# bpatchasaheb/mayaMatchMoveSolver

Hardware: AMD Instinct MI355X
Metric: LM iterations/sec + residuals/sec (markers x frames) at 1/2/4/8 MI355X; final RMS reproj error (higher is better)
Workload: dtype f64; 1 GPU; c4_500pose_50kbnd_200kobs; frames=500, cameras=1, bundles=50000, markers=50000, observations=200000, parameters=152991, residuals=400000, parallelism=single, solver=lmder fwd-FD delta=1e-4 tau=1 tol=1e-6

## Files before the change

include/mmba.h:

```cpp
#ifndef MMBA_H
#define MMBA_H

#include <stddef.h>
#include <stdint.h>

#ifdef __cplusplus
extern "C" {
#endif

#define MMBA_ABI_VERSION 12

#define MMBA_OK 0
#define MMBA_ERR_INVALID (-1)
#define MMBA_ERR_DEVICE (-2)
#define MMBA_ERR_UNSUPPORTED (-3)
#define MMBA_ERR_INTERRUPTED (-4)
#define MMBA_ERR_NO_DEVICE (-5)
#define MMBA_ERR_COMM (-6)

#define MMBA_SOLVER_CMINPACK_LMDIF 1
#define MMBA_SOLVER_CMINPACK_LMDER 2

#define MMBA_SCENE_GRAPH_MAYA_DAG 1
#define MMBA_SCENE_GRAPH_MM_SCENE_GRAPH 2
// ... 226 lines not shown

typedef struct mmba_error_metrics {
    int32_t *frame_count;
    double *frame_avg;
    double *frame_max;
    int32_t *frame_max_marker;
    int32_t *marker_count;
    double *marker_avg;
    double *marker_max;
    int32_t *marker_max_frame;
} mmba_error_metrics;
int mmba_plan_error_metrics(mmba_plan *plan, mmba_error_metrics *out);

int mmba_plan_param_layout(const mmba_plan *plan, int32_t *class_out, int32_t *block_out);

int mmba_solve_per_frame(mmba_context *ctx, const mmba_problem *prob,
                         const mmba_options *opt, double *x_inout,
                         mmba_result *results , int32_t max_concurrency,
                         const mmba_callbacks *cb);

int mmba_plan_solve_per_frame(mmba_plan *plan, double *x_inout, mmba_result *results,
                              const mmba_callbacks *cb);

int mmba_solve(mmba_context *ctx, const mmba_problem *prob,
               const mmba_options *opt, double *x_inout, double *fvec_out,
               double *err_user_out, double *err_dist_out, mmba_result *res,
               const mmba_callbacks *cb, mmba_trace *trace);

typedef struct mmba_kernel_stats {
    double jac_ms_avg;
    double jac_bytes;
    int32_t jac_launches;
    double resid_ms_avg;
    double resid_bytes;
    int32_t resid_launches;
    double chol_ms_avg;
    double chol_flops;
    int32_t chol_launches;
    int32_t reduced_dim;
    int32_t reduced_kind;
    int32_t dataflow_fallback;
    int32_t shards_replicated;
    int32_t spec_replays;
    int32_t band_solver;
    int32_t band_levels;
    int32_t band_block;
    double chol_flops_alg;
    int32_t pre_handbacks;
    int32_t ne_split_launches;
    int32_t trial_red_folds;
} mmba_kernel_stats;
int mmba_plan_kernel_stats(mmba_plan *plan, int enable_timing,
                           mmba_kernel_stats *out);

#define MMBA_PATH_PCR 1
#define MMBA_PATH_SHARD_BCR 2
#define MMBA_PATH_BCR_DATAFLOW 3
#define MMBA_PATH_BCR_GRID 4
#define MMBA_PATH_DENSE 5
#define MMBA_PATH_PERFRAME_BATCH 6
#define MMBA_PATH_LOCAL_RING 7
#define MMBA_PATH_PROBE 8
#define MMBA_PATH_SHARD_SEP 9
#define MMBA_PATH_TRIAL_RECORDS 10
#define MMBA_PATH_LENS_CF 11
#define MMBA_PATH_DEST_LANE 12
#define MMBA_PATH_FAULT_SHARD 13
#define MMBA_PATH_COMM_TIMEOUT_MS 14
#define MMBA_PATH_STALL_SHARD 15
#define MMBA_PATH_PCR_CHAIN 16
#define MMBA_PATH_BACKSUB_ONEPASS 17
#define MMBA_PATH_JB_RECOMPUTE 18
#define MMBA_PATH_NE_CF_SPLIT 19
#define MMBA_PATH_RED_BD 20
#define MMBA_PATH_HANDBACK_DMA 21
#define MMBA_PATH_PRE_HANDBACK 22
#define MMBA_PATH_PRE_SCHUR 23
#define MMBA_PATH_BACKSUB_GROUP 24
#define MMBA_PATH_TRIAL_RED_FOLD 25
#define MMBA_PATH_LENS_SHARED 26
#define MMBA_PATH_OBJ_CF 27
#define MMBA_PATH_OBJ_REC 28
#define MMBA_PATH_PCR_WIDE 29
#define MMBA_PATH_NUM 30
int mmba_debug_set_path(int key, int value);

int mmba_debug_band_solve(mmba_context *ctx, int nb, int w, int nG, int P, const double *S,
                          const double *r, double *x, double *ynorm2, int *parts_used);
int mmba_debug_comm_allreduce(mmba_context *ctx, mmba_comm *comm, double *buf, int count,
                              int op);
int mmba_debug_dgemm(mmba_context *ctx, int tri, int in_place, int M, int N, int K,
                     const double *A, int lda, const double *B, int ldb, double *C, int ldc,
                     double alpha, double beta);

int mmba_debug_reduced_residual(mmba_plan *plan, const double *x, double lam, double *relres);

int mmba_debug_damped_step(mmba_plan *plan, const double *x, double lam, double *step_out,
                           double *g_out, double *diag_out, double *fjac_out);

int mmba_debug_error_metrics(mmba_context *ctx, int32_t num_frames, int32_t num_markers,
                             int32_t num_obs, const int32_t *obs_marker,
                             const int32_t *obs_frame, const double *err_dist,
                             mmba_error_metrics *out);

#ifdef __cplusplus
}
#endif

#endif
```

mayamatchmovesolver_amd/abi.py:

```python
import ctypes as C

MMBA_OK = 0
MMBA_ERR_INVALID = -1
MMBA_ERR_DEVICE = -2
MMBA_ERR_UNSUPPORTED = -3
MMBA_ERR_INTERRUPTED = -4
MMBA_ERR_NO_DEVICE = -5
MMBA_ERR_COMM = -6

SOLVER_TYPE_CMINPACK_LMDIF = 1
SOLVER_TYPE_CMINPACK_LMDER = 2
SCENE_GRAPH_MODE_MAYA_DAG = 1
SCENE_GRAPH_MODE_MM_SCENE_GRAPH = 2
AUTO_DIFF_TYPE_FORWARD = 0
AUTO_DIFF_TYPE_CENTRAL = 1
ROBUST_LOSS_TYPE_TRIVIAL = 0
ROBUST_LOSS_TYPE_SOFT_L_ONE = 1
ROBUST_LOSS_TYPE_CAUCHY = 2
ABI_VERSION = 12

PATH_PCR = 1
PATH_SHARD_BCR = 2
PATH_BCR_DATAFLOW = 3
PATH_BCR_GRID = 4
PATH_DENSE = 5
PATH_PERFRAME_BATCH = 6
PATH_LOCAL_RING = 7
PATH_PROBE = 8
PATH_SHARD_SEP = 9
PATH_TRIAL_RECORDS = 10
PATH_LENS_CF = 11
PATH_DEST_LANE = 12
PATH_FAULT_SHARD = 13
PATH_COMM_TIMEOUT_MS = 14
PATH_STALL_SHARD = 15
PATH_PCR_CHAIN = 16
PATH_BACKSUB_ONEPASS = 17
PATH_JB_RECOMPUTE = 18
PATH_NE_CF_SPLIT = 19
PATH_RED_BD = 20
PATH_HANDBACK_DMA = 21
PATH_PRE_HANDBACK = 22
PATH_PRE_SCHUR = 23
PATH_BACKSUB_GROUP = 24
PATH_TRIAL_RED_FOLD = 25
PATH_LENS_SHARED = 26
PATH_OBJ_CF = 27
PATH_OBJ_REC = 28
PATH_PCR_WIDE = 29
PATH_NUM = 30

FILM_FIT_FILL = 0
FILM_FIT_HORIZONTAL = 1
FILM_FIT_VERTICAL = 2
FILM_FIT_OVERSCAN = 3

ROO_XYZ, ROO_YZX, ROO_ZXY, ROO_XZY, ROO_YXZ, ROO_ZYX = range(6)

LENS_NONE = 0
LENS_3DE_CLASSIC = 1
LENS_3DE_RADIAL_STD_DEG4 = 2
LENS_3DE_ANAMORPHIC_STD_DEG4 = 3
LENS_3DE_ANAMORPHIC_STD_DEG4_RESCALED = 4

CAM_FILM_BACK_W_INCH = 0
CAM_FILM_BACK_H_INCH = 1
CAM_FOCAL_MM = 2
CAM_FILM_OFFSET_X_INCH = 3
CAM_FILM_OFFSET_Y_INCH = 4
CAM_NEAR_CLIP = 5
CAM_FAR_CLIP = 6
CAM_SCALE = 7
CAM_NUM_ATTRS = 8
LENS_NUM_ATTRS = 14

_i32p = C.POINTER(C.c_int32)
_i64p = C.POINTER(C.c_int64)
_f64p = C.POINTER(C.c_double)


class MmbaProblem(C.Structure):
    _fields_ = [
        ("num_frames", C.c_int32),
        ("num_attrs", C.c_int32),
        ("attr_animated", _i32p),
        ("attr_offset", _i64p),
        ("attr_values", _f64p),
        ("num_transforms", C.c_int32),
        ("tfm_parent", _i32p),
        ("tfm_rotate_order", _i32p),
        ("tfm_attrs", _i32p),
        ("num_cameras", C.c_int32),
        ("cam_tfm", _i32p),
        ("cam_attrs", _i32p),
        ("cam_film_fit", _i32p),
        ("cam_render_size", _i32p),
        ("cam_lens", _i32p),
        ("num_lenses", C.c_int32),
        ("lens_type", _i32p),
        ("lens_attrs", _i32p),
        ("num_bundles", C.c_int32),
        ("bnd_tfm", _i32p),
        ("num_markers", C.c_int32),
        ("mkr_cam", _i32p),
        ("mkr_bnd", _i32p),
        ("num_obs", C.c_int32),
        ("obs_marker", _i32p),
        ("obs_frame", _i32p),
        ("obs_xy", _f64p),
        ("obs_weight", _f64p),
        ("num_params", C.c_int32),
        ("param_attr", _i32p),
        ("param_frame", _i32p),
        ("param_min", _f64p),
        ("param_max", _f64p),
        ("param_offset", _f64p),
        ("param_scale", _f64p),
        ("param_weight", _f64p),
        ("num_stiff", C.c_int32),
        ("stiff_attr", _i32p),
        ("stiff_frame", _i32p),
        ("stiff_weight", _f64p),
        ("stiff_variance", _f64p),
        ("stiff_value", _f64p),
        ("num_smooth", C.c_int32),
        ("smooth_attr", _i32p),
        ("smooth_frame", _i32p),
        ("smooth_weight", _f64p),
        ("smooth_variance", _f64p),
        ("smooth_value", _f64p),
        ("cam_rs_value", _f64p),
        ("lens_input", _i32p),
        ("lens_input_values", _f64p),
# ... 166 lines not shown
```

mayamatchmovesolver_amd/csrc/mmba_api.cpp:

```cpp
#include <atomic>
#include <cfloat>
#include <cmath>
#include <cstring>
#include <string>

#include "mmba_geom.h"
#include "mmba_kernels.h"
#include "mmba_plan.h"

namespace mmba {
static thread_local std::string g_last_error;
void set_error(const std::string &msg) { g_last_error = msg; }

static_assert(MMBA_PATH_NUM == 30, "one initialiser per path key");
static std::atomic<int> g_path[MMBA_PATH_NUM] = {-1, -1, -1, -1, -1, -1, -1, -1, -1, -1, -1, -1, -1,
                                                 -1, -1, -1, -1, -1, -1, -1, -1, -1, -1, -1, -1,
                                                 -1, -1, -1, -1, -1};
int path_choice(int key) {
    return (key > 0 && key < MMBA_PATH_NUM) ? g_path[key].load() : -1;
}
}

using namespace mmba;

#define MMBA_GUARD(...)                               \
    try {                                             \
        __VA_ARGS__                                   \
    } catch (const DeviceError &) {                   \
        return MMBA_ERR_DEVICE;                       \
    } catch (const CommError &) {                     \
        return MMBA_ERR_COMM;                         \
    } catch (const Unsupported &u) {                  \
        set_error("unsupported: " + u.what);          \
        return MMBA_ERR_UNSUPPORTED;                  \
    } catch (const Invalid &v) {                      \
        set_error("invalid: " + v.what);              \
        return MMBA_ERR_INVALID;                      \
    } catch (const std::exception &e) {               \
        set_error(std::string("exception: ") + e.what()); \
        return MMBA_ERR_INVALID;                      \
    }

extern "C" {

int mmba_abi_version(void) { return MMBA_ABI_VERSION; }

int mmba_debug_set_path(int key, int value) {
    if (key <= 0 || key >= MMBA_PATH_NUM) return MMBA_ERR_INVALID;
    g_path[key].store(value < 0 ? -1 : value);
    return MMBA_OK;
}

int mmba_shard_layout(int32_t num_frames, int32_t num_obs, const int32_t *obs_frame,
                      const int32_t *obs_bundle, int32_t num_bundles, int32_t nranks,
                      int32_t *bounds_out, int32_t *bundle_owner_out) {
    if (num_frames <= 0 || num_obs < 0 || nranks <= 0 || !bounds_out ||
        (num_obs > 0 && !obs_frame) || (bundle_owner_out && (!obs_bundle || num_bundles < 0)))
        return MMBA_ERR_INVALID;
    for (int i = 0; i < num_obs; ++i) {
        if (obs_frame[i] < 0 || obs_frame[i] >= num_frames) return MMBA_ERR_INVALID;
        if (bundle_owner_out && (obs_bundle[i] < 0 || obs_bundle[i] >= num_bundles))
            return MMBA_ERR_INVALID;
    }
    mmba::shard_layout(num_frames, num_obs, obs_frame, obs_bundle, num_bundles, nranks,
                       bounds_out, bundle_owner_out);
    return MMBA_OK;
}

const char *mmba_last_error(void) { return g_last_error.c_str(); }

int mmba_device_count(void) {
    int count = 0;
    if (hipGetDeviceCount(&count) != hipSuccess) return 0;
    int ok = 0;
    for (int d = 0; d < count; ++d) {
        hipDeviceProp_t prop;
        if (hipGetDeviceProperties(&prop, d) != hipSuccess) continue;
        if (std::strncmp(prop.gcnArchName, "gfx950", 6) == 0) ++ok;
    }
    return ok;
}

void mmba_options_default(mmba_options *o, int32_t solver_type) {
    if (!o) return;
    std::memset(o, 0, sizeof(*o));
    o->solver_type = solver_type ? solver_type : MMBA_SOLVER_CMINPACK_LMDER;
    o->iter_max = 100;
    o->tau = 1.0;
    o->eps1 = 1e-6;
    o->eps2 = 1e-6;
    o->eps3 = 1e-6;
    o->delta = 1e-4;
    o->auto_diff_type = MMBA_AUTO_DIFF_FORWARD;
    o->auto_param_scale = 1;
    o->scene_graph_mode = MMBA_SCENE_GRAPH_MAYA_DAG;
    o->image_width = 2048.0;
    o->accept_only_better = 1;
    o->log_level = 0;
}

// ... 576 lines not shown
```

mayamatchmovesolver_amd/csrc/mmba_internal.h:

```cpp
#pragma once

#include <hip/hip_runtime.h>
#include <stdint.h>

#include <string>
#include <vector>

#include "../../include/mmba.h"

namespace mmba {

constexpr int PCMAX = 12;
constexpr int PBMAX = 3;
constexpr int NGMAX = 48;
constexpr int NGLANE = 16;
constexpr int NGPART = 32;
constexpr int LMAX = 32;
constexpr int CF_AIDX = 16;
constexpr int TILE = 64;
constexpr int CAMREC = 20;
constexpr int LENS_LAYER = 1 + MMBA_LENS_NUM_ATTRS;
constexpr int LENS_CHAIN_MAX = 4;
constexpr int BREC = 16;
constexpr int ORECSZ = 12;
// ... 100 lines not shown
    int s_xn2 = 0, s_gnorm = 0, s_f0 = 0, s_out = 0;
    int *gate = nullptr;
};
struct BandSolver {
    bool use_bd = false;
    BdDev bd;
    bool use_bcr = false;
    BcrDev bcr;
    bool use_pcr = false;
    PcrDev pcr;
    mutable unsigned tick_f = 0, tick_b = 0;
    mutable bool df_off = false;
    int df_grid = 256;
    double *red = nullptr, *red_rhs = nullptr;
    size_t red_count = 0;
    int P = 1, w = 0, nb = 0, nG = 0;
    int p_lo = 0, p_hi = 1;
    Comm *comm = nullptr;
    long long max_arrow = 0;
    double *Bd = nullptr, *Ga = nullptr, *Gd = nullptr, *Gdinv = nullptr, *Dinv = nullptr;
    BandPart *d_parts = nullptr;
    double *apool = nullptr, *zpool = nullptr, *cpool = nullptr;
    double *TBd = nullptr, *TGa = nullptr, *TGd = nullptr, *TGdinv = nullptr, *TDinv = nullptr;
    size_t tcount = 0;
    BandPart *d_tpart = nullptr;
    double *rT = nullptr, *yT = nullptr, *xT = nullptr;
    bool pcr_int = false;
    PcrDev ipcr;
    BandPart hpart{};
    double *XA = nullptr, *izero = nullptr, *ix = nullptr;
    int *fail = nullptr;
};

struct SView {
    int band;
    int dense, ld;
    double *S;
    const int *slot;
    int NT;
    double *Bd;
    int w, nb;
    double *Ga;
    double *Gd;
};

enum ParamClass : int { PC_CF = 0, PC_B = 1, PC_G = 2 };

enum VarFlags : int { VF_BUNDLE_SIDE = 1, VF_LENS = 2, VF_OBJ = 4 };

struct DevProblem {
    int F, nA, nT, nC, nL, nB, nK, M, n, ncf, nR, nG, mode;
    int nbs;
    double image_width;
    const int64_t *attr_off;
    const int *attr_anim;
    double *attr_val;
    const int *tfm_parent, *tfm_roo, *tfm_attrs;
    const int *cam_tfm, *cam_attrs, *cam_fit, *cam_size, *cam_lens;
    const int *lens_attrs, *lens_type;
    const double *lens_chain;
    int lens_chain_n;
    int lens_uniform;
    const int *bnd_tfm;
    const int *obs_cf, *obs_bnd, *obs_frame, *obs_cam;
    const double *obs_xy, *obs_sqrtw;
    const int *cf_cam, *cf_frame, *cf_obs_off, *cf_var_off, *cf_var_param, *cf_var_flags;
    const int *cf_pc, *cf_roff;
    int pc_uniform;
    int wst;
    int dest_diag_ii;
    const int *bnd_par_off, *bnd_par;
    const int *bnd_pb;
    const int *bnd_xoff;
    const int *bobs_off, *bobs;
    const int4 *bnd_p4;
    const double *brec;
    int all_bnd_fast;
    int lmax;
    int jcol_implicit;
    const int *cf_aidx;
    int no_lens;
    const int *obs_bpos;
    double *JB;
    const int *cam_lpar_off, *cam_lpar;
    const int *obs_inst, *inst_lens, *inst_attr, *inst_frame, *inst_lpar_off, *inst_lpar;
    const double *inst_val;
    const int *p_attr, *p_frame, *p_class, *p_pos, *p_both, *p_blk;
    const double *p_min, *p_max, *p_off, *p_scale;
    const int *g_param;
    const int *obs_own, *cf_own, *bnd_own;
    int root, Ra, Rb;
    int nrows, rows_live;
    const int *row_attr, *row_frame, *row_param;
    const double *row_w, *row_var, *row_val;
    int loss_on, loss_type;
    double loss_scale;
    const long long *p_vidx;
    const int4 *bnd_vx;
    const int *bnd_pcomp;
    int rs;
    const double *obs_tau;
    const int *cf_rs_nb, *cf_rs_vidx;
    const int *cf_rs_gcnt, *cf_rs_gcol, *cf_rs_gidx;
    double *rs_Aoff;
    int ls_ng, ls_nl;
    const int *ls_tab;
    double *ls_Aoff;
};

struct ObjRecDev {
    int n = 0;
    const int *obs_set = nullptr, *off = nullptr, *par = nullptr, *set = nullptr, *tf = nullptr;
    double *rec = nullptr;
};
struct NoObjRec {};

__device__ __forceinline__ size_t widx(const DevProblem &P, int k, int i) {
    return (size_t)i * P.wst + k;
}

__device__ __forceinline__ double *s_at(const SView &V, int R, int C) {
    if (V.dense) return &V.S[(size_t)C * V.ld + R];
    if (!V.band) {
        const int s = V.slot[(R / TILE) * V.NT + (C / TILE)];
        return &V.S[(size_t)s * TILE * TILE + (R % TILE) * TILE + (C % TILE)];
    }
    if (R < V.nb) return &V.Bd[(size_t)R * (V.w + 1) + (C - R + V.w)];
    if (C < V.nb) return &V.Ga[(size_t)(R - V.nb) * V.nb + C];
    return &V.Gd[(R - V.nb) * NGMAX + (C - V.nb)];
}

}
```

mayamatchmovesolver_amd/csrc/mmba_kernels.h:

```cpp
#pragma once

#include <vector>

#include "mmba_internal.h"

namespace mmba {

constexpr int NE_BND_TPB = 64;

inline int nblk(long n, int bs) { return (int)((n + bs - 1) / bs); }

void launch_param_set(hipStream_t s, const DevProblem &P, const double *x, double *ext,
                      double *ext_pert, double *step, int solver_type, double delta,
                      double eps_dif);
struct RedRow {
    int off, n, is_max, slot;
};
struct RedSpec {
    int nrows;
    int flag_slot;
    RedRow row[8];
};
void launch_reduce_multi(hipStream_t s, const double *partial, const RedSpec &spec,
                         double *scalar, int *flag = nullptr, double *host = nullptr,
// ... 21 lines not shown
                          const double *recs, double *f, double *eu, double *ed, double *partial,
                          double *out, unsigned int *ticket, double *dist);
void launch_residual_jp_orec(hipStream_t s, const DevProblem &P, const ObjRecDev &O,
                             const double *recs, double *f, double *eu, double *ed,
                             double *partial, const double *J, const int *jcol, const int *nloc,
                             const double *pstep, double *partial_jp, double *dist);
void launch_jacobian_orec(hipStream_t s, const DevProblem &P, const ObjRecDev &O,
                          const double *recs, const double *ext_pert, const double *step,
                          int solver_type, double *J, int *jcol, int *nloc,
                          const int *stale_param, double *eu, double *ed);
int residual_blocks(const DevProblem &P);
bool &trial_cf_off();
int trial_blocks(const DevProblem &P);
void launch_reproject(hipStream_t s, const DevProblem &P, const double *recs, double *pts,
                      double *mkr);
void launch_residual(hipStream_t s, const DevProblem &P, const double *recs, double *f, double *eu,
                     double *ed, double *partial, double *out = nullptr,
                     unsigned int *ticket = nullptr, double *dist = nullptr,
                     const ObjRecDev *O = nullptr);
void launch_dist_stats(hipStream_t s, const DevProblem &P, const double *ed, double *partial,
                       int nparts, int rstride, double *out);
void launch_residual_jp(hipStream_t s, const DevProblem &P, const double *recs, double *f,
                        double *eu, double *ed, double *partial, const double *J,
                        const int *jcol, const int *nloc, const double *pstep,
                        double *partial_jp, double *dist = nullptr,
                        const ObjRecDev *O = nullptr);
struct CentralB {
    const double *recs = nullptr, *brec = nullptr, *ext_pert = nullptr, *step = nullptr;
    const double *q15 = nullptr, *kap15 = nullptr;
};
void launch_param_central(hipStream_t s, const DevProblem &P, const double *x, double *ext_pertB,
                          double *stepB, double delta, double *count, double *c15 = nullptr);
void launch_b15_s(hipStream_t s, const double *fsq, double fn, double *out);
void launch_b15_combine(hipStream_t s, int n, const double *u, const double *c, const double *zu,
                        const double *zc, const double *sp, double *xs, double *kinv,
                        double *scalar, int fail_slot, const double *fail_prev);
void launch_b15_q(hipStream_t s, const DevProblem &P, const double *c, double *q15, double *kap15,
                  double *cr);
void launch_b15_rot(hipStream_t s, const DevProblem &P, const double *q15, const double *x,
                    double *out);
void launch_b15_accl(hipStream_t s, const DevProblem &P, const double *Acc, const double *q15,
                     const double *diag, double lam, double *AccL, double *diagL);
void launch_b15_unrot(hipStream_t s, const DevProblem &P, const double *Acc, const double *g,
                      const double *q15, double *adiag, double *u);
void launch_b15_unrot_J(hipStream_t s, const DevProblem &P, double *J, const double *q15);
void launch_b15_dnorm(hipStream_t s, int n, const double *x, const double *diag, double *out);
void launch_b15_newton(hipStream_t s, int n, const double *v, const double *zu, const double *zc,
                       const double *kinv, double *out);
void launch_b15_jp(hipStream_t s, int n, const double *xs, const double *u, const double *c,
                   const double *sp, double *out);
void launch_jacobian(hipStream_t s, const DevProblem &P, const double *recs,
                     const double *ext_pert, const double *step, int solver_type, double *J,
                     int *jcol, int *nloc, const int *stale_param, double *eu, double *ed,
                     int ncv = 0,
                     const double *f = nullptr,
                     const CentralB &CB = CentralB(),
                     const ObjRecDev *O = nullptr);
void launch_rows_eval(hipStream_t s, const DevProblem &P, double *fr, double *eur,
                      double *partial, int slot, const double *Jrow = nullptr,
                      const double *pstep = nullptr, double *partial_jp = nullptr);
void launch_rows_jac(hipStream_t s, const DevProblem &P, const double *ext,
                     const double *ext_pert, const double *step, const double *ext_pertB,
                     const double *stepB, int lmder, double *Jrow, double *eur, int last_param);
void launch_rows_ne(hipStream_t s, const DevProblem &P, const double *Jrow, const double *fr,
                    const int *p_own, double *Acc, double *Abb, double *aggbuf, double *g);
constexpr int NE_CF_SPLIT = 4;
constexpr int NE_CF_NT = 36;
struct NeEpi {
    int on = 0;
    int first = 0, mode = 1, do_xn = 0, do_gn = 0;
    double fnorm = 0.;
    const double *fnorm_sq = nullptr;
    const double *x = nullptr;
    double *diag = nullptr, *acnorm = nullptr, *partial = nullptr;
    int rstride = 0, cf_base = 0, bnd_base = 0;
    const double *jb_recs = nullptr;
    int jb_lmder = 1;
    double *cf_part = nullptr;
    unsigned *cf_ticket = nullptr;
    double *Lb = nullptr, *tb = nullptr;
    int *fail = nullptr;
    const int *gate = nullptr;
    long long *probe = nullptr;
};
struct TrialRed {
    int on = 0;
    RedSpec spec{};
    LmDec dec{};
    const double *partial = nullptr;
    double *scalar = nullptr;
    double *host = nullptr;
    int host_n = 0;
    unsigned *host_seq = nullptr;
    unsigned seq = 0;
};
bool jac_ne_fusable(const DevProblem &P, int ncv);
void launch_jac_ne(hipStream_t s, const DevProblem &P, const double *recs, const double *step,
                   int solver_type, double *J, int *jcol, int *nloc, const int *stale_param,
                   double *eu, double *ed, double *Acc, double *g, const NeEpi &E,
                   const TrialRed &R = TrialRed());
bool ne_epilogue_fusable(const DevProblem &P);
bool launch_ne(hipStream_t s, const DevProblem &P, const double *J, const int *jcol,
               const int *nloc, const double *f, double *Acc, double *Acg, double *Abb,
               double *Abg, double *aggbuf, double *g, double *glob_partial, int glob_chunk,
               const NeEpi &epi = NeEpi(), bool cf_done = false);
void launch_colnorms(hipStream_t s, const DevProblem &P, const double *Acc, const double *Abb,
                     const double *aggbuf, double *acnorm, double *g);
void launch_bundle_factor(hipStream_t s, const DevProblem &P, const double *Abb,
                          const double *Abg, const double *g, const double *diag, double lam,
                          double *Lb, double *tb, double *Wg, int *fail);
void launch_schur_obs(hipStream_t s, const DevProblem &P, const double *J, const double *Lb,
                      double *W, const RedSpec *red = nullptr, const double *partial = nullptr,
                      double *scalar = nullptr, const int *gate = nullptr);
void launch_schur_obs_rs(hipStream_t s, const DevProblem &PV, int Mr, const int *nloc,
                         const int *vobs, const int *vcoff, const double *J, const double *Lb,
                         double *W);
void launch_schur_init(hipStream_t s, const DevProblem &P, const double *Acc, const double *Acg,
                       const double *Agg, const double *g, const double *diag, double lam,
                       const SView &V, int npad, double *rhs, const RedSpec *red = nullptr,
                       const double *partial = nullptr, double *scalar = nullptr);
void launch_schur_pairs(hipStream_t s, const DevProblem &P, const double *W, const double *Wg,
                        const double *tb, const SView &V, double *rhs);
void launch_chol_panel(hipStream_t s, double *S, const int *slot, int NT, int k, const int *rows,
                       int nrows, double *Linv, int *fail);
void launch_chol_update(hipStream_t s, double *S, const int *slot, int NT, int k,
                        const int2 *pairs, int npairs);
void launch_trsv_fwd(hipStream_t s, const double *S, const int *slot, int NT, int k,
                     const int *rows, int nrows, const double *Linv, double *r, double *y);
void launch_trsv_bwd(hipStream_t s, const double *S, const int *slot, int NT, int k,
                     const int *cols, int ncols, const double *Linv, double *y, double *x);
void launch_trsv_fwd_all(hipStream_t s, const double *S, const int *slot, int NT,
                         const int *rows_off, const int *rows, const double *Linv, double *r,
                         double *y);
void launch_trsv_bwd_all(hipStream_t s, const double *S, const int *slot, int NT,
                         const int *cols_off, const int *cols, const double *Linv, double *y,
                         double *x);
struct SchurInitFold {
    int on;
    const double *Acc, *g, *diag;
    double lam;
};
bool launch_schur_dest(hipStream_t s, const DevProblem &P, const double *W, const int2 *dest,
                       const int *dest_off, int ndest, const int2 *pairs, const SView &V,
                       int pc_uniform, int assign_off, const double *tb = nullptr,
                       double *rhs = nullptr, SchurInitFold fold = SchurInitFold{},
                       const int *wave_list = nullptr, int n_wave = 0,
                       const int *lane_list = nullptr, int n_lane = 0);
void launch_schur_rhs(hipStream_t s, const DevProblem &P, const double *W, const double *tb,
                      double *rhs);
void launch_schur_glob(hipStream_t s, const DevProblem &P, const double *W, const double *Wg,
                       const double *tb, const SView &V, double *rhs);
void launch_backsub_bundle(hipStream_t s, const DevProblem &P, const double *W, const double *Wg,
                           const double *tb, const double *Lb, const double *xR, double *U,
                           double *x);
struct TrialFold {
    const double *x = nullptr, *diag = nullptr;
    double *wa1 = nullptr, *wa2 = nullptr, *wa3 = nullptr;
    double *ext = nullptr, *ext_pert = nullptr, *step = nullptr;
    int solver_type = 0;
    double delta = 0., eps_dif = 0.;
    const int *other = nullptr;
    int nother = 0;
    double *partial = nullptr;
    int rstride = 0;
    const int *own = nullptr;
    int rec = 0;
    double *recs = nullptr, *brec = nullptr;
    int group = 0;
    const int2 *bobs_rp = nullptr;
    int brec_fwd = 0;
    int *flag = nullptr;
    double *flag_out = nullptr;
};
bool trial_records_ok(const DevProblem &P);
int trial_fold_parts(const DevProblem &P, int nother, bool rec = false);
int trial_prep_rec_parts(const DevProblem &P, int nother);
void launch_trial_prep_rec(hipStream_t s, const DevProblem &P, const double *xs, const TrialFold &T);
void launch_obs_wtx(hipStream_t s, const DevProblem &P, const double *W, const double *xR,
                    double *U);
void launch_backsub_trial(hipStream_t s, const DevProblem &P, const double *W, const double *Wg,
                          const double *tb, const double *Lb, const double *xR, const double *U,
                          double *x, const TrialFold &T);
void launch_scatter_xR(hipStream_t s, const DevProblem &P, const double *xR, double *x);
void launch_newton_bundle(hipStream_t s, const DevProblem &P, const double *W, const double *Wg,
                          const double *Lb, const double *v, double *wR, double *usq,
                          double *un, double *gp);
void launch_gather_R(hipStream_t s, const DevProblem &P, const double *v, double *vR, int nRpad);
void band_factor(hipStream_t s, const BandSolver &B, int *fail, long long *probe);
void band_factor_forward(hipStream_t s, const BandSolver &B, int *fail, long long *probe,
                         const double *r, double *y);
void band_forward(hipStream_t s, const BandSolver &B, const double *r, double *y);
void band_backward(hipStream_t s, const BandSolver &B, const double *y, double *x);
void bcr_factor(hipStream_t s, const BandSolver &B, int *fail, long long *probe,
                const double *r = nullptr, double *y = nullptr);
void bcr_forward(hipStream_t s, const BandSolver &B, const double *r, double *y);
void bcr_backward(hipStream_t s, const BandSolver &B, const double *y, double *x);
// ... 69 lines not shown
```

mayamatchmovesolver_amd/csrc/mmba_kernels.hip:

```cpp
#include <cfloat>
#include <cstdlib>
#include <type_traits>

#include "mmba_geom.h"
#include "mmba_kernels.h"
#include "mmba_obs_dev.h"
#include "mmba_red_dev.h"

namespace mmba {

__device__ __forceinline__ void bundle_chol3(double (&A)[3][3], double (&rhs)[3],
                                             const double (&dd)[3], int pb, double lam, int b,
                                             double *Lb, double *tb, int *fail,
                                             double (*Lo)[3] = nullptr, double *ilo = nullptr) {
#pragma unroll
    for (int a = 0; a < 3; ++a) {
        if (a < pb) {
            const double d = dd[a];
            A[a][a] += lam * (d * d);
            if (A[a][a] == 0.) {
                A[a][a] = 1.;
                rhs[a] = 0.;
            }
        }
// ... 599 lines not shown
            for (int t = threadIdx.x; t < lm * NE_CHUNK; t += blockDim.x) {
                const int l = t / NE_CHUNK, o = t % NE_CHUNK;
                if (o >= cnt || l < pc || l >= nloc[c0 + o]) continue;
                const int p = jcol[(size_t)l * M + c0 + o];
                if (P.p_class[p] == PC_G) sG[P.p_pos[p] - nCF][o] = l;
            }
        }
        for (int t = threadIdx.x; t < NE_CHUNK; t += blockDim.x) {
            sF[0][t] = (t < cnt) ? f[2 * (c0 + t)] : 0.;
            sF[1][t] = (t < cnt) ? f[2 * (c0 + t) + 1] : 0.;
        }
        __syncthreads();
        if (kind == 0) {
            for (int o = 0; o < cnt; ++o)
                acc += sJ[2 * ea][o] * sJ[2 * eb][o] + sJ[2 * ea + 1][o] * sJ[2 * eb + 1][o];
        } else if (kind == 1) {
            for (int o = 0; o < cnt; ++o)
                acc += sJ[2 * ea][o] * sF[0][o] + sJ[2 * ea + 1][o] * sF[1][o];
        } else if (kind == 2) {
            for (int o = 0; o < cnt; ++o) {
                const int l = sG[eb][o];
                if (l >= 0)
                    acc += sJ[2 * ea][o] * sJ[2 * l][o] + sJ[2 * ea + 1][o] * sJ[2 * l + 1][o];
            }
        }
    }
    double *A = &Acc[(size_t)cf * PCMAX * PCMAX];
    if (kind == 0) {
        A[ea * PCMAX + eb] = acc;
        A[eb * PCMAX + ea] = acc;
    } else if (kind == 1) {
        g[P.cf_var_param[P.cf_var_off[cf] + 1 + ea]] = acc;
    } else if (kind == 2) {
        Acg[((size_t)cf * PCMAX + ea) * NGMAX + eb] = acc;
    }
}

__device__ __forceinline__ double epi_param(const NeEpi &E, int p, double d, double gp, double &zf,
                                          double &xn, double &gm) {
    const double an = sqrt(d);
    E.acnorm[p] = an;
    double dg = E.diag[p];
    if (E.mode != 2) {
        if (E.first) dg = an == 0. ? 1. : an;
        dg = fmax(dg, an);
        E.diag[p] = dg;
    }
    if (an == 0.) zf = 1.;
    if (E.do_xn) {
        const double v = dg * E.x[p];
        xn += v * v;
    }
    if (E.do_gn && an != 0.) {
        const double fn = E.fnorm_sq ? sqrt(*E.fnorm_sq) : E.fnorm;
        if (fn != 0.) gm = fmax(gm, fabs((gp / fn) / an));
    }
    return dg;
}

__device__ __forceinline__ void epi_store(const NeEpi &E, int col, double zf, double xn,
                                          double gm) {
    E.partial[col] = zf;
    E.partial[E.rstride + col] = xn;
    E.partial[2 * E.rstride + col] = gm;
}

struct EpiPre {
    int p;
    double dg;
    double xv;
    double fn;
};
template <int PC>
__device__ __forceinline__ EpiPre epi_preload(const DevProblem &P, const NeEpi &E, int cf,
                                              int lane, bool own = false, double fsq_own = 0.) {
    EpiPre q{-1, 0., 0., 0.};
    if (!E.on || lane >= PC) return q;
    q.p = P.cf_var_param[P.cf_var_off[cf] + 1 + lane];
    q.dg = E.diag[q.p];
    if (E.do_xn) q.xv = E.x[q.p];
    if (E.do_gn) q.fn = own ? sqrt(fsq_own) : E.fnorm_sq ? sqrt(*E.fnorm_sq) : E.fnorm;
    return q;
}
__device__ __forceinline__ void epi_param_pre(const NeEpi &E, const EpiPre &q, double d, double gp,
                                              double &zf, double &xn, double &gm) {
    const double an = sqrt(d);
    E.acnorm[q.p] = an;
    double dg = q.dg;
    if (E.mode != 2) {
        if (E.first) dg = an == 0. ? 1. : an;
        dg = fmax(dg, an);
        E.diag[q.p] = dg;
    }
    if (an == 0.) zf = 1.;
    if (E.do_xn) {
        const double v = dg * q.xv;
        xn += v * v;
    }
    if (E.do_gn && an != 0.) {
        if (q.fn != 0.) gm = fmax(gm, fabs((gp / q.fn) / an));
    }
}
template <int PC>
__device__ __forceinline__ void epi_params_wave(const DevProblem &P, const NeEpi &E, int cf,
                                                int lane, double d, double gp, const EpiPre &q) {
    double zf = 0., xn = 0., gm = 0.;
    if (lane < PC) epi_param_pre(E, q, d, gp, zf, xn, gm);
    double Z = 0., X = 0., G = 0.;
#pragma unroll
    for (int a = 0; a < PC; ++a) {
        const double za = __shfl(zf, a), xa = __shfl(xn, a), ga = __shfl(gm, a);
        if (za != 0.) Z = 1.;
        X += xa;
        G = fmax(G, ga);
    }
    if (lane == 0) epi_store(E, E.cf_base + cf, Z, X, G);
}


template <int PC, int NW, int NG>
__device__ __forceinline__ void ne_cf_u_body(const DevProblem &P, const double *__restrict__ J,
                                             const int *__restrict__ jcol,
                                             const int *__restrict__ nloc,
                                             const double *__restrict__ f, double *Acc,
                                             double *Acg, double *g, const NeEpi &E, int blk,
                                             int nblk_cf) {
    constexpr int NCC = PC * (PC + 1) / 2, NE = NCC + PC, NT = NE + PC * NG;
    __shared__ double wsum[NW][NT];
    const int cf = xcd_remap(blk, nblk_cf);
    if (!own_cf(P, cf) || P.cf_pc[cf] != PC) {
        if (E.on && threadIdx.x == 0) epi_store(E, E.cf_base + cf, 0., 0., 0.);
        return;
    }
    const int o0 = P.cf_obs_off[cf], o1 = P.cf_obs_off[cf + 1];
    const size_t M = P.M;
    const int nCF = P.nR - P.nG;
    const int tid = threadIdx.x, lane = tid & 63, wv = tid >> 6;
    const EpiPre epq = epi_preload<PC>(P, E, cf, lane);
    double acc[NT];
#pragma unroll
    for (int e = 0; e < NT; ++e) acc[e] = 0.;
    for (int i = o0 + tid; i < o1; i += 64 * NW) {
        double jx[PC], jy[PC];
#pragma unroll
        for (int a = 0; a < PC; ++a) {
            jx[a] = J[(2 * a) * M + i];
            jy[a] = J[(2 * a + 1) * M + i];
        }
        const double fx = f[2 * i], fy = f[2 * i + 1];
        int e = 0;
#pragma unroll
        for (int a = 0; a < PC; ++a)
#pragma unroll
            for (int c = a; c < PC; ++c) acc[e++] += jx[a] * jx[c] + jy[a] * jy[c];
#pragma unroll
        for (int a = 0; a < PC; ++a) acc[NCC + a] += jx[a] * fx + jy[a] * fy;
        if constexpr (NG > 0) {
            double gx[NG], gy[NG];
#pragma unroll
            for (int q = 0; q < NG; ++q) gx[q] = gy[q] = 0.;
            const int nl = nloc[i];
            for (int l = PC; l < nl; ++l) {
                const int p = jcol[(size_t)l * M + i];
                if (P.p_class[p] != PC_G) continue;
                const int gi = P.p_pos[p] - nCF;
                const double ux = J[(size_t)(2 * l) * M + i], uy = J[(size_t)(2 * l + 1) * M + i];
#pragma unroll
                for (int q = 0; q < NG; ++q) {
                    gx[q] = (gi == q) ? ux : gx[q];
                    gy[q] = (gi == q) ? uy : gy[q];
                }
            }
#pragma unroll
            for (int a = 0; a < PC; ++a)
#pragma unroll
                for (int q = 0; q < NG; ++q)
                    acc[NE + a * NG + q] += jx[a] * gx[q] + jy[a] * gy[q];
        }
    }
#pragma unroll
    for (int e = 0; e < NT; ++e) {
        double v = acc[e];
#pragma unroll
        for (int off = 32; off > 0; off >>= 1) v += __shfl_xor(v, off);
// ... 137 lines not shown
template <int PC, int NW, int NG>
__global__ void __launch_bounds__(64 * NW) k_ne_cf_u(DevProblem P, const double *__restrict__ J,
                                                     const int *__restrict__ jcol,
                                                     const int *__restrict__ nloc,
                                                     const double *__restrict__ f, double *Acc,
                                                     double *Acg, double *g, NeEpi E) {
    ne_cf_u_body<PC, NW, NG>(P, J, jcol, nloc, f, Acc, Acg, g, E, blockIdx.x, gridDim.x);
}



__device__ __forceinline__ void jac_ne_publish(const TrialRed &R, const LmIn &v, const LmOut &o) {
    if (threadIdx.x == 0) {
        const double val[5] = {v.pnorm, v.xn2t, v.fnorm, v.jp, v.dnorm};
#pragma unroll
        for (int r = 0; r < 5; ++r)
            if (r < R.spec.nrows) R.scalar[R.spec.row[r].slot] = val[r];
        lm_publish(R.dec, o, R.scalar);
    }
    if (!R.host) return;
    if (threadIdx.x < 64) {
        __builtin_amdgcn_fence(__ATOMIC_SEQ_CST, "workgroup");
        for (int i = threadIdx.x; i < R.host_n; i += 64)
            R.host[i] = __hip_atomic_load(&R.scalar[i], __ATOMIC_RELAXED, __HIP_MEMORY_SCOPE_AGENT);
        if (R.host_seq) {
            __threadfence_system();
            if (threadIdx.x == 0)
                __hip_atomic_store(R.host_seq, R.seq, __ATOMIC_RELEASE, __HIP_MEMORY_SCOPE_SYSTEM);
        }
    }
}

struct TrialRows {
    RowQ Q0, Q1;
    int r0, nred;
    bool dn_dup;
};
template <int NW>
__device__ __forceinline__ void trial_rows_issue(const TrialRed &R, LmIn &tin, TrialRows &T) {
    const LmDec &d = R.dec;
    const int nr = R.spec.nrows;
    T.dn_dup = nr == 5 && R.spec.row[4].off == R.spec.row[0].off &&
               R.spec.row[4].n == R.spec.row[0].n &&
               R.spec.row[4].is_max == R.spec.row[0].is_max;
    T.nred = T.dn_dup ? 4 : nr;
    T.r0 = __builtin_amdgcn_readfirstlane((int)threadIdx.x >> 6);
    if (T.r0 < T.nred) row_issue(R.partial, R.spec.row[T.r0], T.Q0);
    if constexpr (NW == 2)
        if (T.r0 + NW < T.nred) row_issue(R.partial, R.spec.row[T.r0 + NW], T.Q1);
    tin.f0 = R.scalar[d.s_f0];
    tin.xn2 = R.scalar[d.s_xn2];
    tin.gnorm = R.scalar[d.s_gnorm];
    tin.fail = R.scalar[d.s_fail];
    if (nr < 5) tin.dnorm = R.scalar[d.s_dnorm];
}
template <int NW>
__device__ __forceinline__ void trial_rows_finish(const TrialRed &R, double *sTr,
                                                  const TrialRows &T) {
    const bool l0 = (threadIdx.x & 63) == 0;
    if (T.r0 < T.nred) {
        const double v = row_finish(R.partial, R.spec.row[T.r0], T.Q0);
        if (l0) sTr[T.r0] = v;
    }
    if constexpr (NW == 2)
        if (T.r0 + NW < T.nred) {
            const double v = row_finish(R.partial, R.spec.row[T.r0 + NW], T.Q1);
            if (l0) sTr[T.r0 + NW] = v;
        }
    for (int r = T.r0 + (NW == 2 ? 2 : 1) * NW; r < T.nred; r += NW) {
        const double v = reduce_row_w64(R.partial, R.spec.row[r]);
        if (l0) sTr[r] = v;
    }
}
__device__ __forceinline__ LmOut trial_decide(const TrialRed &R, const double *sTr, LmIn &tin,
                                              bool dn_dup) {
    tin.pnorm = sTr[0];
    tin.xn2t = sTr[1];
    tin.fnorm = sTr[2];
    tin.jp = sTr[3];
    if (R.spec.nrows == 5) tin.dnorm = dn_dup ? sTr[0] : sTr[4];
    return lm_decide_vals(R.dec, tin);
}

template <int PC, int NW, bool GEN>
__global__ void __launch_bounds__(64 * NW) k_jac_ne_u(
    DevProblem P, const double *__restrict__ recs, const double *__restrict__ step,
    int solver_type, double *__restrict__ J, int *__restrict__ jcol, int *__restrict__ nloc,
    const int *__restrict__ stale_param, double *__restrict__ eu, double *__restrict__ ed,
    double *Acc, double *g, NeEpi E, TrialRed R) {
    constexpr int NCC = PC * (PC + 1) / 2, NE = NCC + PC;
    __shared__ double wsum[NW][NE];
    __shared__ double sRec[(PC + 1) * CAMREC];
    __shared__ int sPv[PC];
    __shared__ double sSt[PC];
    __shared__ int sHdr[3];
    __shared__ double sTr[5];
    if (!R.on && E.gate &&
        __hip_atomic_load(E.gate, __ATOMIC_RELAXED, __HIP_MEMORY_SCOPE_AGENT) == 0)
        return;
    const int tid = threadIdx.x, lane = tid & 63, wv = tid >> 6;
    LmIn tin{};
    TrialRows TR;
    TR.dn_dup = false;
    const int pad = R.on ? 8 : 0;
    const int ncf = (int)gridDim.x - pad;
    if ((int)blockIdx.x < pad) {
        if (blockIdx.x != 0) return;
        trial_rows_issue<NW>(R, tin, TR);
        trial_rows_finish<NW>(R, sTr, TR);
        __syncthreads();
        const LmOut out = trial_decide(R, sTr, tin, TR.dn_dup);
        jac_ne_publish(R, tin, out);
        return;
    }
    const int cf = xcd_remap((int)blockIdx.x - pad, ncf);
    long long *pr = (E.probe && threadIdx.x == 0) ? E.probe + 5 * (size_t)cf : nullptr;
    const long long t_in = pr ? (long long)wall_clock64() : 0;
    const int o0 = P.cf_obs_off[cf], o1 = P.cf_obs_off[cf + 1];
    const bool lmder = solver_type == MMBA_SOLVER_CMINPACK_LMDER;
    const bool solved = P.cf_pc[cf] == PC && own_cf(P, cf);
    {
        constexpr int KT = ((PC + 1) * CAMREC + 64 * NW - 1) / (64 * NW);
        const int voff = P.cf_var_off[cf];
        const int nv = min(P.cf_var_off[cf + 1] - voff - 1, PC);
        double rv[KT];
#pragma unroll
        for (int k = 0; k < KT; ++k) {
            const int t = tid + 64 * NW * k;
            rv[k] = t < (nv + 1) * CAMREC ? recs[(size_t)voff * CAMREC + t] : 0.;
        }
        const int p = (tid < PC && tid < nv) ? P.cf_var_param[voff + 1 + tid] : -1;
        const int fr = P.cf_frame[cf];
        if (R.on) trial_rows_issue<NW>(R, tin, TR);
        const double stv = p >= 0 ? step[p] : 1.;
#pragma unroll
        for (int k = 0; k < KT; ++k) {
            const int t = tid + 64 * NW * k;
            if (t < (nv + 1) * CAMREC) sRec[t] = rv[k];
        }
        if (tid < PC) {
            sPv[tid] = p;
            sSt[tid] = stv;
        }
        if (tid == 0) {
            sHdr[0] = nv;
            sHdr[1] = fr;
            sHdr[2] = stale_param[fr];
        }
    }
    if (R.on) trial_rows_finish<NW>(R, sTr, TR);
    __syncthreads();
    if (R.on && trial_decide(R, sTr, tin, TR.dn_dup).go == 0) return;
    if (pr) {
        pr[0] = t_in;
        pr[1] = (long long)wall_clock64();
    }
    JacCf<PC> C;
    C.rcf = sRec;
#pragma unroll
    for (int v = 0; v < PC; ++v) {
        C.pv[v] = sPv[v];
        C.st[v] = sSt[v];
    }
    C.nv = sHdr[0];
    C.fr = sHdr[1];
    C.pstale = sHdr[2];
    double acc[NE];
#pragma unroll
    for (int e = 0; e < NE; ++e) acc[e] = 0.;
    for (int i = o0 + tid; i < o1; i += 64 * NW) {
        double jx[PC], jy[PC], fx, fy;
        int z = 0;
        asm volatile("" : "+s"(z));
        C.rcf = sRec + z;
        jac_obs_u<PC, GEN>(P, i, C, lmder, J, jcol, nloc, eu, ed, jx, jy, fx, fy);
        int e = 0;
#pragma unroll
        for (int a = 0; a < PC; ++a)
#pragma unroll
            for (int c = a; c < PC; ++c) acc[e++] += jx[a] * jx[c] + jy[a] * jy[c];
#pragma unroll
        for (int a = 0; a < PC; ++a) acc[NCC + a] += jx[a] * fx + jy[a] * fy;
    }
    if (pr) pr[2] = (long long)wall_clock64();
    if (!solved) {
        if (E.on && tid == 0) epi_store(E, E.cf_base + cf, 0., 0., 0.);
        if (pr) pr[3] = pr[2];
        return;
    }
#pragma unroll
    for (int e = 0; e < NE; ++e) {
        double v = acc[e];
#pragma unroll
        for (int off = 32; off > 0; off >>= 1) v += __shfl_xor(v, off);
        if (lane == 0) wsum[wv][e] = v;
    }
    __syncthreads();
    double *A = &Acc[(size_t)cf * PCMAX * PCMAX];
    for (int e = tid; e < NE; e += 64 * NW) {
        double v = wsum[0][e];
#pragma unroll
        for (int w = 1; w < NW; ++w) v += wsum[w][e];
        if (e < NCC) {
            int a = 0, rem = e;
            while (rem >= PC - a) {
                rem -= PC - a;
                ++a;
            }
            const int c = a + rem;
            A[a * PCMAX + c] = v;
            A[c * PCMAX + a] = v;
        } else {
            g[P.cf_var_param[P.cf_var_off[cf] + 1 + (e - NCC)]] = v;
        }
    }
    if (E.on && (tid >> 6) == 0) {
        const int ln = tid & 63;
        double d = 0., gp = 0.;
        if (ln < PC) {
            const int ed2 = ln * PC - ln * (ln - 1) / 2;
            d = wsum[0][ed2];
            gp = wsum[0][NCC + ln];
#pragma unroll
            for (int w = 1; w < NW; ++w) {
                d += wsum[w][ed2];
                gp += wsum[w][NCC + ln];
            }
        }
        epi_params_wave<PC>(P, E, cf, ln, d, gp, epi_preload<PC>(P, E, cf, ln, R.on != 0, sTr[2]));
    }
    if (pr) {
        pr[3] = (long long)wall_clock64();
        unsigned xcc;
        asm volatile("s_getreg_b32 %0, hwreg(HW_REG_XCC_ID)" : "=s"(xcc));
        pr[4] = (long long)(xcc & 0xf);
    }
}

__global__ void __launch_bounds__(NE_BND_TPB) k_ne_bnd_jb(DevProblem P, double *Abb, double *g,
                                                          NeEpi E) {
    __shared__ double red[3][NE_BND_TPB];
    if (E.gate && __hip_atomic_load(E.gate, __ATOMIC_RELAXED, __HIP_MEMORY_SCOPE_AGENT) == 0)
        return;
    const int b = xcd_remap(blockIdx.x, gridDim.x) * blockDim.x + threadIdx.x;
    const int4 p4 = b < P.nB ? P.bnd_p4[b] : make_int4(-1, -1, -1, 0);
    const int pb = p4.w;
    double zf = 0., xn = 0., gm = 0.;
    if (pb > 0) {
        double A[PBMAX][PBMAX] = {};
        double gb[PBMAX] = {};
        const int q0 = P.bobs_off[b], q1 = P.bobs_off[b + 1];
        const double *__restrict__ br = &P.brec[(size_t)b * BREC];
        for (int qb = q0; qb < q1; qb += 4) {
            double4 u[4], v[4];
            if (E.jb_recs) {
                const double bp0[3] = {br[0], br[1], br[2]};
#pragma unroll
                for (int r = 0; r < 4; ++r) {
                    if (qb + r >= q1) break;
                    const int i = P.bobs[qb + r];
                    const double *__restrict__ rec0 = &E.jb_recs[(size_t)P.cf_var_off[P.obs_cf[i]] * CAMREC];
                    const double mx = P.obs_xy[2 * i], my = P.obs_xy[2 * i + 1], sw = P.obs_sqrtw[i];
                    const double2 f0 = residual_e(rec0, bp0, mx, my, sw, P.mode, P.image_width);
                    double jb[6] = {0., 0., 0., 0., 0., 0.};
#pragma unroll
                    for (int a = 0; a < 3; ++a) {
                        if (a < pb) {
                            const double bq[3] = {br[3 + 3 * a], br[4 + 3 * a], br[5 + 3 * a]};
                            const double2 rr = residual_e(rec0, bq, mx, my, sw, P.mode, P.image_width);
                            const double st = br[12 + a];
                            jb[2 * a] = E.jb_lmder ? (rr.x - f0.x) * st : (rr.x - f0.x) / st;
                            jb[2 * a + 1] = E.jb_lmder ? (rr.y - f0.y) * st : (rr.y - f0.y) / st;
                        }
                    }
                    u[r] = make_double4(jb[0], jb[1], jb[2], jb[3]);
                    v[r] = make_double4(jb[4], jb[5], f0.x, f0.y);
                }
            } else {
#pragma unroll
                for (int r = 0; r < 4; ++r) {
                    if (qb + r < q1) {
                        const double4 *src = reinterpret_cast<const double4 *>(&P.JB[(size_t)(qb + r) * 8]);
                        u[r] = src[0];
                        v[r] = src[1];
                    }
                }
            }
#pragma unroll
            for (int r = 0; r < 4; ++r) {
                if (qb + r >= q1) break;
                const double jx[3] = {u[r].x, u[r].z, v[r].x}, jy[3] = {u[r].y, u[r].w, v[r].y};
                const double fx = v[r].z, fy = v[r].w;
#pragma unroll
                for (int a = 0; a < 3; ++a) {
#pragma unroll
                    for (int c = 0; c < 3; ++c) A[a][c] += jx[a] * jx[c] + jy[a] * jy[c];
                    gb[a] += jx[a] * fx + jy[a] * fy;
                }
            }
        }
        double *Ab = &Abb[(size_t)b * 9];
#pragma unroll
        for (int a = 0; a < PBMAX; ++a)
#pragma unroll
            for (int c = 0; c < PBMAX; ++c) Ab[a * 3 + c] = (a < pb && c < pb) ? A[a][c] : 0.;
        g[p4.x] = gb[0];
        if (pb > 1) g[p4.y] = gb[1];
        if (pb > 2) g[p4.z] = gb[2];
        double dd[3] = {0., 0., 0.};
        if (E.on) {
            double zo = 0., xo = 0., go = 0.;
            dd[0] = epi_param(E, p4.x, A[0][0], gb[0], zo, xo, go);
            if (pb > 1) dd[1] = epi_param(E, p4.y, A[1][1], gb[1], zo, xo, go);
            if (pb > 2) dd[2] = epi_param(E, p4.z, A[2][2], gb[2], zo, xo, go);
            if (own_bnd(P, b)) {
                zf = zo;
                xn = xo;
                gm = go;
            }
        }
        if (E.Lb) {
            double Af[3][3], rhs[3];
#pragma unroll
            for (int a = 0; a < 3; ++a) {
#pragma unroll
                for (int c = 0; c < 3; ++c)
                    Af[a][c] = (a < pb && c < pb) ? A[a][c] : (a == c ? 1. : 0.);
                rhs[a] = a < pb ? gb[a] : 0.;
            }
            bundle_chol3(Af, rhs, dd, pb, 0.0, b, E.Lb, E.tb, E.fail);
        }
    }
    if (!E.on) return;
    red[0][threadIdx.x] = zf;
    red[1][threadIdx.x] = xn;
    red[2][threadIdx.x] = gm;
    __syncthreads();
    for (int w = NE_BND_TPB / 2; w > 0; w >>= 1) {
        if (threadIdx.x < w) {
            red[0][threadIdx.x] = fmax(red[0][threadIdx.x], red[0][threadIdx.x + w]);
            red[1][threadIdx.x] += red[1][threadIdx.x + w];
            red[2][threadIdx.x] = fmax(red[2][threadIdx.x], red[2][threadIdx.x + w]);
        }
        __syncthreads();
    }
    if (threadIdx.x == 0) {
        const int col = E.bnd_base + xcd_remap(blockIdx.x, gridDim.x);
        epi_store(E, col, red[0][0], red[1][0], red[2][0]);
    }
}

__global__ void k_ne_bnd(DevProblem P, const double *__restrict__ J,
                         const int *__restrict__ jcol, const int *__restrict__ nloc,
                         const double *__restrict__ f, double *Abb, double *Abg, double *g) {
    const int b = blockIdx.x * blockDim.x + threadIdx.x;
    if (b >= P.nB) return;
    const int pb = P.bnd_pb[b];
    if (pb == 0) return;
    const int M = P.M, nG = P.nG;
    double A[PBMAX][PBMAX] = {};
    double gb[PBMAX] = {};
    double G[PBMAX][NGMAX];
    for (int a = 0; a < PBMAX; ++a)
        for (int q = 0; q < NGMAX; ++q) G[a][q] = 0.;
    for (int q = P.bobs_off[b]; q < P.bobs_off[b + 1]; ++q) {
        const int i = P.bobs[q];
        const int cf = P.obs_cf[i];
        const int s = P.rs ? nloc[i] - pb : P.cf_var_off[cf + 1] - P.cf_var_off[cf] - 1;
        double jx[PBMAX], jy[PBMAX];
        for (int a = 0; a < pb; ++a) {
            jx[a] = J[(size_t)(2 * (s + a)) * M + i];
            jy[a] = J[(size_t)(2 * (s + a) + 1) * M + i];
        }
        const double fx = f[2 * i], fy = f[2 * i + 1];
        for (int a = 0; a < pb; ++a) {
            for (int c = 0; c < pb; ++c) A[a][c] += jx[a] * jx[c] + jy[a] * jy[c];
            gb[a] += jx[a] * fx + jy[a] * fy;
        }
        if (nG > 0) {
            const int nl = nloc[i];
            for (int l = 0; l < nl; ++l) {
                const int p = jcol[(size_t)l * M + i];
                if (P.p_class[p] != PC_G) continue;
                const int gi = P.p_pos[p] - (P.nR - nG);
                const double gx = J[(size_t)(2 * l) * M + i], gy = J[(size_t)(2 * l + 1) * M + i];
                for (int a = 0; a < pb; ++a) G[a][gi] += jx[a] * gx + jy[a] * gy;
            }
        }
    }
    double *Ab = &Abb[(size_t)b * 9];
    for (int a = 0; a < PBMAX; ++a)
        for (int c = 0; c < PBMAX; ++c) Ab[a * 3 + c] = (a < pb && c < pb) ? A[a][c] : 0.;
    const int po = P.bnd_par_off[b];
    for (int a = 0; a < pb; ++a) g[P.bnd_par[po + a]] = gb[a];
    for (int a = 0; a < PBMAX; ++a)
        for (int q = 0; q < nG; ++q) Abg[((size_t)b * PBMAX + a) * NGMAX + q] = G[a][q];
}
// ... 314 lines not shown
                                                      double *host, int host_n,
                                                      unsigned *ticket, unsigned *host_seq,
                                                      unsigned seq, const LmDec dec) {
    __shared__ double red[256];
    const RedRow rw = spec.row[blockIdx.x];
    const double v = reduce_row_block<false>(partial, rw, red);
    if (threadIdx.x == 0) {
        scalar[rw.slot] = v;
        if (blockIdx.x == 0 && flag && spec.flag_slot >= 0) {
            scalar[spec.flag_slot] = (double)*flag;
            *flag = 0;
        }
    }
    if (!host && !dec.on) return;
    __shared__ unsigned last;
    if (threadIdx.x == 0) {
        const unsigned t = __hip_atomic_fetch_add(ticket, 1u, __ATOMIC_ACQ_REL,
                                                  __HIP_MEMORY_SCOPE_AGENT);
        last = t == gridDim.x - 1;
    }
    __syncthreads();
    if (!last) return;
    __builtin_amdgcn_fence(__ATOMIC_ACQUIRE, "agent");
    if (dec.on) {
        if (threadIdx.x == 0) lm_decide(dec, scalar);
        __syncthreads();
        __builtin_amdgcn_fence(__ATOMIC_SEQ_CST, "workgroup");
    }
    if (!host) {
        if (threadIdx.x == 0)
            __hip_atomic_store(ticket, 0u, __ATOMIC_RELAXED, __HIP_MEMORY_SCOPE_AGENT);
        return;
    }
    if (threadIdx.x < 64) {
        for (int i = threadIdx.x; i < host_n; i += 64)
            host[i] = __hip_atomic_load(&scalar[i], __ATOMIC_RELAXED, __HIP_MEMORY_SCOPE_AGENT);
        if (host_seq) {
            __threadfence_system();
            if (threadIdx.x == 0)
                __hip_atomic_store(host_seq, seq, __ATOMIC_RELEASE, __HIP_MEMORY_SCOPE_SYSTEM);
        }
    }
    if (threadIdx.x == 0) __hip_atomic_store(ticket, 0u, __ATOMIC_RELAXED, __HIP_MEMORY_SCOPE_AGENT);
}

__global__ void k_bundle_factor(DevProblem P, const double *__restrict__ Abb,
                                const double *__restrict__ Abg, const double *__restrict__ g,
                                const double *__restrict__ diag, double lam, double *Lb,
                                double *tb, double *Wg, int *fail) {
    const int b = xcd_remap(blockIdx.x, gridDim.x) * blockDim.x + threadIdx.x;
    if (b >= P.nB) return;
    const int pb = P.bnd_pb[b];
    if (pb == 0) return;
    const int po = P.bnd_par_off[b];
    double A[3][3], rhs[3], dd[3];
#pragma unroll
    for (int a = 0; a < 3; ++a) {
#pragma unroll
        for (int c = 0; c < 3; ++c)
            A[a][c] = (a < pb && c < pb) ? Abb[(size_t)b * 9 + a * 3 + c] : (a == c ? 1. : 0.);
        rhs[a] = 0.;
        dd[a] = 0.;
        if (a < pb) {
            const int p = P.bnd_par[po + a];
            dd[a] = diag[p];
            rhs[a] = g[p];
        }
    }
    double L[3][3], il[3];
    bundle_chol3(A, rhs, dd, pb, lam, b, Lb, tb, fail, L, il);
    for (int q = 0; q < P.nG; ++q) {
        double w[3];
#pragma unroll
        for (int a = 0; a < 3; ++a) {
            double s = a < pb ? Abg[((size_t)b * PBMAX + a) * NGMAX + q] : 0.;
#pragma unroll
            for (int k = 0; k < a; ++k) s -= L[a][k] * w[k];
            w[a] = s * il[a];
        }
        for (int a = 0; a < 3; ++a) Wg[((size_t)b * NGMAX + q) * 3 + a] = w[a];
    }
}

template <int PCT>
__global__ void __launch_bounds__(64) k_schur_obs(DevProblem P, const double *__restrict__ J,
                                                  const double *__restrict__ Lb, double *W,
                                                  int nob, const RedSpec red,
                                                  const double *__restrict__ partial,
                                                  double *scalar, const int *gate) {
    extern __shared__ double sw[];
    if (gate && __hip_atomic_load(gate, __ATOMIC_RELAXED, __HIP_MEMORY_SCOPE_AGENT) == 0) return;
    const int lane = threadIdx.x;
    if ((int)blockIdx.x >= nob) {
        const RedRow rw = red.row[blockIdx.x - nob];
        const double v = reduce_row_w64(partial, rw);
        if (lane == 0) scalar[rw.slot] = v;
        return;
    }
    const int i0 = xcd_remap(blockIdx.x, nob) * 64;
    const int i = i0 + lane;
    const int M = P.M, wst = P.wst;
    double *row = &sw[lane * wst];
    for (int k = 0; k < wst; ++k) row[k] = 0.;
    const int b = i < M ? P.obs_bnd[i] : 0;
    const int pb = i < M ? P.bnd_pb[b] : 0;
    if (pb > 0) {
        const int cf = P.obs_cf[i];
        const int pc = min(min(P.cf_pc[cf], wst / 3), PCT);
        const int s = P.cf_var_off[cf + 1] - P.cf_var_off[cf] - 1;
        double bx[3], by[3], L[3][3], il[3];
#pragma unroll
        for (int a = 0; a < 3; ++a) {
            bx[a] = a < pb ? J[(size_t)(2 * (s + a)) * M + i] : 0.;
            by[a] = a < pb ? J[(size_t)(2 * (s + a) + 1) * M + i] : 0.;
#pragma unroll
            for (int c = 0; c < 3; ++c) L[a][c] = Lb[(size_t)b * 9 + a * 3 + c];
        }
#pragma unroll
        for (int a = 0; a < 3; ++a) il[a] = a < pb ? 1.0 / L[a][a] : 0.;
        double cx[PCT], cy[PCT];
#pragma unroll
        for (int r = 0; r < PCT; ++r) {
            cx[r] = r < pc ? J[(size_t)(2 * r) * M + i] : 0.;
            cy[r] = r < pc ? J[(size_t)(2 * r + 1) * M + i] : 0.;
        }
#pragma unroll
        for (int r = 0; r < PCT; ++r) {
            if (r < pc) {
                double w[3];
#pragma unroll
                for (int a = 0; a < 3; ++a) {
                    double t = cx[r] * bx[a] + cy[r] * by[a];
#pragma unroll
                    for (int k = 0; k < a; ++k) t -= L[a][k] * w[k];
                    w[a] = t * il[a];
                }
#pragma unroll
                for (int a = 0; a < 3; ++a) row[r * 3 + a] = w[a];
            }
        }
    }
    __syncthreads();
    const int nrow = min(64, M - i0);
    const size_t base = (size_t)i0 * wst;
    if (wst % 2 == 0) {
        const int nv = nrow * wst / 2;
        double2 *dst = reinterpret_cast<double2 *>(&W[base]);
        const double2 *src = reinterpret_cast<const double2 *>(sw);
        for (int k = lane; k < nv; k += 64) dst[k] = src[k];
    } else {
        for (int k = lane; k < nrow * wst; k += 64) W[base + k] = sw[k];
    }
}

__global__ void __launch_bounds__(64) k_schur_obs_rs(DevProblem PV, int Mr,
                                                     const int *__restrict__ nloc,
                                                     const int *__restrict__ vobs,
                                                     const int *__restrict__ vcoff,
                                                     const double *__restrict__ J,
                                                     const double *__restrict__ Lb, double *W) {
    const int v = blockIdx.x * blockDim.x + threadIdx.x;
    if (v >= PV.M) return;
    const int wst = PV.wst;
    double *row = &W[(size_t)v * wst];
    for (int k = 0; k < wst; ++k) row[k] = 0.;
    const int b = PV.obs_bnd[v];
    const int pb = PV.bnd_pb[b];
    if (pb <= 0) return;
    const int i = vobs[v], cf = PV.obs_cf[v];
    const int pc = min(PV.cf_pc[cf], wst / 3);
    const int c0 = vcoff[v], s = nloc[i] - pb;
    double bx[3], by[3], L[3][3], il[3];
#pragma unroll
    for (int a = 0; a < 3; ++a) {
        bx[a] = a < pb ? J[(size_t)(2 * (s + a)) * Mr + i] : 0.;
        by[a] = a < pb ? J[(size_t)(2 * (s + a) + 1) * Mr + i] : 0.;
#pragma unroll
        for (int c = 0; c < 3; ++c) L[a][c] = Lb[(size_t)b * 9 + a * 3 + c];
    }
#pragma unroll
    for (int a = 0; a < 3; ++a) il[a] = a < pb ? 1.0 / L[a][a] : 0.;
    for (int r = 0; r < pc; ++r) {
        const double cx = J[(size_t)(2 * (c0 + r)) * Mr + i], cy = J[(size_t)(2 * (c0 + r) + 1) * Mr + i];
        double w[3];
#pragma unroll
        for (int a = 0; a < 3; ++a) {
            double t = cx * bx[a] + cy * by[a];
#pragma unroll
            for (int k = 0; k < a; ++k) t -= L[a][k] * w[k];
            w[a] = t * il[a];
        }
#pragma unroll
        for (int a = 0; a < 3; ++a) row[r * 3 + a] = w[a];
    }
}

__device__ __forceinline__ void schur_init_row(
    const DevProblem &P, const double *__restrict__ Acc, const double *__restrict__ Acg,
    const double *__restrict__ Agg, const double *__restrict__ g,
// ... 1406 lines not shown
        nmn = fmax(nmn, partial[rstride + i]);
        mx = fmax(mx, partial[2 * rstride + i]);
    }
    red[0][threadIdx.x] = sm;
    red[1][threadIdx.x] = nmn;
    red[2][threadIdx.x] = mx;
    __syncthreads();
    for (int w = 128; w > 0; w >>= 1) {
        if ((int)threadIdx.x < w) {
            red[0][threadIdx.x] += red[0][threadIdx.x + w];
            red[1][threadIdx.x] = fmax(red[1][threadIdx.x], red[1][threadIdx.x + w]);
            red[2][threadIdx.x] = fmax(red[2][threadIdx.x], red[2][threadIdx.x + w]);
        }
        __syncthreads();
    }
    if (threadIdx.x == 0) {
        out[0] = red[0][0];
        out[1] = red[1][0];
        out[2] = red[2][0];
    }
}

void launch_dist_stats(hipStream_t s, const DevProblem &P, const double *ed, double *partial,
                       int nparts, int rstride, double *out) {
    k_dist_stats<<<nparts, 256, 0, s>>>(P, ed, partial, rstride);
    k_dist_stats_fin<<<1, 256, 0, s>>>(partial, nparts, rstride, out);
}
void launch_jacobian(hipStream_t s, const DevProblem &P, const double *recs,
                     const double *ext_pert, const double *step, int solver_type, double *J,
                     int *jcol, int *nloc, const int *stale_param, double *eu, double *ed,
                     int ncv, const double *f, const CentralB &CB, const ObjRecDev *O) {
    (void)f;
    if (P.rs) {
        launch_jacobian_rs(s, P, ext_pert, step, solver_type, J, jcol, nloc, stale_param, eu, ed);
        return;
    }
    constexpr bool uni = true;
#define MMBA_JAC_U(NCV, GEN)                                                                \
    do {                                                                                    \
        if (uni)                                                                            \
            k_jacobian_u<NCV, GEN, true><<<nblk(P.M, 128), 128, 0, s>>>(                    \
                P, recs, step, solver_type, J, jcol, nloc, stale_param, eu, ed);            \
        else                                                                                \
            k_jacobian_u<NCV, GEN, false><<<nblk(P.M, 128), 128, 0, s>>>(                   \
                P, recs, step, solver_type, J, jcol, nloc, stale_param, eu, ed);            \
    } while (0)
    if (ncv == 6 || ncv == 7) {
        if (ncv == 6) {
            if (P.all_bnd_fast) MMBA_JAC_U(6, false); else MMBA_JAC_U(6, true);
        } else {
            if (P.all_bnd_fast) MMBA_JAC_U(7, false); else MMBA_JAC_U(7, true);
        }
        return;
    }
#undef MMBA_JAC_U
    if (CB.recs)
        k_jacobian<true><<<nblk(P.M, 128), 128, 0, s>>>(P, recs, ext_pert, step, solver_type, J,
                                                      jcol, nloc, stale_param, eu, ed, CB,
                                                      NoObjRec{});
    else if (O && O->n > 0)
        launch_jacobian_orec(s, P, *O, recs, ext_pert, step, solver_type, J, jcol, nloc,
                             stale_param, eu, ed);
    else if (P.lens_uniform == MMBA_LENS_3DE_CLASSIC)
        k_jacobian<false, MMBA_LENS_3DE_CLASSIC><<<nblk(P.M, 128), 128, 0, s>>>(
            P, recs, ext_pert, step, solver_type, J, jcol, nloc, stale_param, eu, ed, CB,
                                                      NoObjRec{});
    else
        k_jacobian<false><<<nblk(P.M, 128), 128, 0, s>>>(P, recs, ext_pert, step, solver_type, J,
                                                       jcol, nloc, stale_param, eu, ed, CB,
                                                      NoObjRec{});
}
bool jac_ne_fusable(const DevProblem &P, int ncv) {
    return P.nG == 0 && P.pc_uniform == ncv && (ncv == 6 || ncv == 7) &&
           P.nrows == 0 && !P.loss_on && P.ncf >= 256 && !P.rs && !P.ls_ng;
}
void launch_jac_ne(hipStream_t s, const DevProblem &P, const double *recs, const double *step,
                   int solver_type, double *J, int *jcol, int *nloc, const int *stale_param,
                   double *eu, double *ed, double *Acc, double *g, const NeEpi &E,
                   const TrialRed &R) {
    if (P.ncf == 0) return;
    const int grid = P.ncf + (R.on ? 8 : 0);
    const long long per = (P.M + P.ncf - 1) / P.ncf;
    int nw = per > 1024 ? 8 : (per > 256 ? 4 : 2);
#define MMBA_JN(PC, NW, GEN)                                                                  \
    k_jac_ne_u<PC, NW, GEN><<<grid, 64 * NW, 0, s>>>(P, recs, step, solver_type, J, jcol, nloc, \
                                                       stale_param, eu, ed, Acc, g, E, R)
#define MMBA_JN_NW(PC, GEN)                                         \
    do {                                                            \
        if (nw == 8) MMBA_JN(PC, 8, GEN);                           \
        else if (nw == 4) MMBA_JN(PC, 4, GEN);                      \
        else MMBA_JN(PC, 2, GEN);                                   \
    } while (0)
#define MMBA_JN_PC(PC)                                              \
    do {                                                            \
        if (P.all_bnd_fast) MMBA_JN_NW(PC, false);                  \
        else MMBA_JN_NW(PC, true);                                  \
    } while (0)
    if (P.pc_uniform == 6)
        MMBA_JN_PC(6);
    else
        MMBA_JN_PC(7);
#undef MMBA_JN_PC
#undef MMBA_JN_NW
#undef MMBA_JN
}
__global__ void k_fold_ranks(const double *__restrict__ t, int nranks, double *out, int do_xn,
                             int do_gn) {
    if (threadIdx.x != 0) return;
    out[0] = t[0];
    if (do_xn) out[1] = t[1];
    if (do_gn) {
        double g = 0.;
        for (int r = 0; r < nranks; ++r) g = fmax(g, t[2 + r]);
        out[2] = g;
    }
}
void launch_fold_ranks(hipStream_t s, const double *t, int nranks, double *out, int do_xn,
                       int do_gn) {
    k_fold_ranks<<<1, 64, 0, s>>>(t, nranks, out, do_xn, do_gn);
}
void launch_param_central(hipStream_t s, const DevProblem &P, const double *x, double *ext_pertB,
                          double *stepB, double delta, double *count, double *c15) {
    if (P.n > 0)
        k_param_central<<<nblk(P.n, 256), 256, 0, s>>>(P, x, ext_pertB, stepB, delta, count,
                                                        c15);
}

template <int NV>
__device__ __forceinline__ void b15_block_sum(double (&v)[NV], double (*red)[1024]) {
    const int tid = threadIdx.x;
#pragma unroll
    for (int k = 0; k < NV; ++k) red[k][tid] = v[k];
    __syncthreads();
    for (int w = 512; w > 0; w >>= 1) {
        if (tid < w) {
#pragma unroll
            for (int k = 0; k < NV; ++k) red[k][tid] += red[k][tid + w];
        }
        __syncthreads();
    }
#pragma unroll
    for (int k = 0; k < NV; ++k) v[k] = red[k][0];
    __syncthreads();
}

__global__ void k_b15_s(const double *fsq, double fn, double *out) {
    if (threadIdx.x == 0) *out = fsq ? *fsq : fn * fn;
}

__global__ void __launch_bounds__(1024) k_b15_combine(
    int n, const double *__restrict__ u, const double *__restrict__ c,
    const double *__restrict__ zu, const double *__restrict__ zc, const double *__restrict__ sp,
    double *xs, double *kinv, double *scalar, int fail_slot, const double *__restrict__ fail_prev) {
    __shared__ double red[4][1024];
    double d[4] = {0., 0., 0., 0.};
    for (int j = threadIdx.x; j < n; j += 1024) {
        d[0] += u[j] * zu[j];
        d[1] += u[j] * zc[j];
        d[2] += c[j] * zu[j];
        d[3] += c[j] * zc[j];
    }
    b15_block_sum<4>(d, red);
    const double s = *sp;
    const double k00 = d[0] - s, k01 = 1. + d[1], k10 = 1. + d[2], k11 = d[3];
    const double det = k00 * k11 - k01 * k10;
    const bool sing = !(fabs(det) > 0.) || !isfinite(det);
    const double i00 = k11 / det, i01 = -k01 / det, i10 = -k10 / det, i11 = k00 / det;
    const double r0 = d[0] + s * d[1], r1 = d[2] + s * d[3];
    const double al = i00 * r0 + i01 * r1, be = i10 * r0 + i11 * r1;
    const double cu = 1. - al, cc = s - be;
    for (int j = threadIdx.x; j < n; j += 1024) xs[j] = cu * zu[j] + cc * zc[j];
    if (threadIdx.x == 0) {
        kinv[0] = i00;
        kinv[1] = i01;
        kinv[2] = i10;
        kinv[3] = i11;
        double f = fmax(scalar[fail_slot], *fail_prev);
        if (sing) f = fmax(f, 1.);
        scalar[fail_slot] = f;
    }
}

__global__ void __launch_bounds__(1024) k_b15_newton(int n, const double *__restrict__ v,
                                                     const double *__restrict__ zu,
                                                     const double *__restrict__ zc,
                                                     const double *__restrict__ kinv, double *out) {
    __shared__ double red[2][1024];
// ... 194 lines not shown
    const int nt = P.n > P.ncf ? P.n : P.ncf;
    if (nt > 0) k_b15_q<<<nblk(nt, 256), 256, 0, s>>>(P, c, q15, kap15, cr);
}
void launch_b15_rot(hipStream_t s, const DevProblem &P, const double *q15, const double *x,
                    double *out) {
    if (P.n > 0) k_b15_rot<<<nblk(P.n, 256), 256, 0, s>>>(P, q15, x, out);
}
void launch_b15_accl(hipStream_t s, const DevProblem &P, const double *Acc, const double *q15,
                     const double *diag, double lam, double *AccL, double *diagL) {
    const int nt = P.n > P.ncf ? P.n : P.ncf;
    if (nt > 0) k_b15_accl<<<nblk(nt, 256), 256, 0, s>>>(P, Acc, q15, diag, lam, AccL, diagL);
}
void launch_b15_unrot(hipStream_t s, const DevProblem &P, const double *Acc, const double *g,
                      const double *q15, double *adiag, double *u) {
    if (P.n > 0) k_b15_unrot<<<nblk(P.n, 256), 256, 0, s>>>(P, Acc, g, q15, adiag, u);
}
void launch_b15_unrot_J(hipStream_t s, const DevProblem &P, double *J, const double *q15) {
    if (P.M > 0) k_b15_unrot_J<<<nblk(P.M, 128), 128, 0, s>>>(P, J, q15);
}
void launch_b15_dnorm(hipStream_t s, int n, const double *x, const double *diag, double *out) {
    k_b15_dnorm<<<1, 1024, 0, s>>>(n, x, diag, out);
}
void launch_b15_newton(hipStream_t s, int n, const double *v, const double *zu, const double *zc,
                       const double *kinv, double *out) {
    k_b15_newton<<<1, 1024, 0, s>>>(n, v, zu, zc, kinv, out);
}
void launch_b15_jp(hipStream_t s, int n, const double *xs, const double *u, const double *c,
                   const double *sp, double *out) {
    k_b15_jp<<<1, 1024, 0, s>>>(n, xs, u, c, sp, out);
}
bool ne_epilogue_fusable(const DevProblem &P) {
    return P.nG == 0 && (P.JB || P.nbs == 0) && (P.pc_uniform == 6 || P.pc_uniform == 7) &&
           !P.rs && !P.ls_ng;
}
bool launch_ne(hipStream_t s, const DevProblem &P, const double *J, const int *jcol,
               const int *nloc, const double *f, double *Acc, double *Acg, double *Abb,
               double *Abg, double *aggbuf, double *g, double *glob_partial, int glob_chunk,
               const NeEpi &epi, bool cf_done) {
    const NeEpi E = ne_epilogue_fusable(P) ? epi : NeEpi();
    double *Agg = aggbuf, *gG = aggbuf + NGMAX * NGMAX;
    bool glob_done = false;
    bool split_done = false;
    if (P.rs) {
        launch_ne_rs(s, P, J, jcol, nloc, f, Acc, Acg, g);
    } else if (P.ncf > 0 && !cf_done) {
        const bool wide = P.M > 1024 * P.ncf || (P.M > 128 * P.ncf && P.ncf < 1024);
#define MMBA_NE_U(PC, NW, NG)                                                              \
    k_ne_cf_u<PC, NW, NG><<<P.ncf, 64 * NW, 0, s>>>(P, J, jcol, nloc, f, Acc, Acg, g, E)
        const int pcu = P.pc_uniform;
        if ((pcu == 6 || pcu == 7) && wide && P.nG > 0 && P.nG <= 2) {
            const int nbg = nblk(P.M, glob_chunk);
            if (pcu == 6)
                k_ne_cf_glob<6><<<P.ncf + nbg, 256, 0, s>>>(P, J, jcol, nloc, f, Acc, Acg, g, E,
                                                           glob_partial, glob_chunk);
            else
                k_ne_cf_glob<7><<<P.ncf + nbg, 256, 0, s>>>(P, J, jcol, nloc, f, Acc, Acg, g, E,
                                                           glob_partial, glob_chunk);
            glob_done = true;
        } else if ((pcu == 6 || pcu == 7) && (P.nG == 0 || P.nG <= 2)) {
            if (P.nG == 0) {
                const bool split = wide && E.cf_part && E.cf_ticket && P.M > 1024 * P.ncf;
                if (split) {
                    split_done = true;
                    const int gs = P.ncf * NE_CF_SPLIT;
                    if (pcu == 6)
                        k_ne_cf_split<6, 4, NE_CF_SPLIT><<<gs, 256, 0, s>>>(P, J, f, Acc, g, E);
                    else
                        k_ne_cf_split<7, 4, NE_CF_SPLIT><<<gs, 256, 0, s>>>(P, J, f, Acc, g, E);
                } else if (pcu == 6) {
                    if (wide) MMBA_NE_U(6, 4, 0); else MMBA_NE_U(6, 1, 0);
                } else {
                    if (wide) MMBA_NE_U(7, 4, 0); else MMBA_NE_U(7, 1, 0);
                }
            } else {
                if (pcu == 6) MMBA_NE_U(6, 1, 2); else MMBA_NE_U(7, 1, 2);
            }
        } else {
            k_ne_cf<<<P.ncf, 256, 0, s>>>(P, J, jcol, nloc, f, Acc, Acg, g);
        }
#undef MMBA_NE_U
    }
    if (P.ls_ng > 0) launch_ne_lens_shared(s, P, J, jcol, nloc, f, Acc, Acg, g);
    if (P.nbs > 0) {
        if (P.JB)
            k_ne_bnd_jb<<<nblk(P.nB, NE_BND_TPB), NE_BND_TPB, 0, s>>>(P, Abb, g, E);
        else
            k_ne_bnd<<<nblk(P.nB, 64), 64, 0, s>>>(P, J, jcol, nloc, f, Abb, Abg, g);
    }
    if (P.nG > 0) {
        const int nb = nblk(P.M, glob_chunk);
        if (glob_done)
            ;
        else if (P.nG <= 2)
            k_ne_glob<2><<<nb, 256, 0, s>>>(P, J, jcol, nloc, f, glob_partial, glob_chunk);
        else if (P.nG <= 4)
            k_ne_glob<4><<<nb, 256, 0, s>>>(P, J, jcol, nloc, f, glob_partial, glob_chunk);
        else if (P.nG <= 8)
            k_ne_glob<8><<<nb, 256, 0, s>>>(P, J, jcol, nloc, f, glob_partial, glob_chunk);
        else if (P.nG <= 16)
            k_ne_glob<16><<<nb, 256, 0, s>>>(P, J, jcol, nloc, f, glob_partial, glob_chunk);
        else
            k_ne_glob_wide<<<nb, 256, 0, s>>>(P, J, jcol, nloc, f, glob_partial, glob_chunk);
        k_ne_glob_reduce<<<1, 256, 0, s>>>(P, glob_partial, nb, Agg, gG);
    }
    return split_done;
}
void launch_colnorms(hipStream_t s, const DevProblem &P, const double *Acc, const double *Abb,
                     const double *aggbuf, double *acnorm, double *g) {
    k_colnorms<<<nblk(P.n, 256), 256, 0, s>>>(P, Acc, Abb, aggbuf, aggbuf + NGMAX * NGMAX,
                                               acnorm, g);
}
void launch_bundle_factor(hipStream_t s, const DevProblem &P, const double *Abb,
                          const double *Abg, const double *g, const double *diag, double lam,
                          double *Lb, double *tb, double *Wg, int *fail) {
    if (P.nB == 0) return;
    k_bundle_factor<<<nblk(P.nB, 64), 64, 0, s>>>(P, Abb, Abg, g, diag, lam, Lb, tb, Wg, fail);
}
void launch_schur_obs(hipStream_t s, const DevProblem &P, const double *J, const double *Lb,
                      double *W, const RedSpec *red, const double *partial, double *scalar,
                      const int *gate) {
    const int nob = nblk(P.M, 64), nr = red ? red->nrows : 0;
    if (nob + nr > 0) {
        if (P.wst / 3 <= 8)
            k_schur_obs<8><<<nob + nr, 64, sizeof(double) * 64 * P.wst, s>>>(
                P, J, Lb, W, nob, red ? *red : RedSpec{}, partial, scalar, gate);
        else
            k_schur_obs<PCMAX><<<nob + nr, 64, sizeof(double) * 64 * P.wst, s>>>(
                P, J, Lb, W, nob, red ? *red : RedSpec{}, partial, scalar, gate);
    }
}
void launch_schur_obs_rs(hipStream_t s, const DevProblem &PV, int Mr, const int *nloc,
                         const int *vobs, const int *vcoff, const double *J, const double *Lb,
                         double *W) {
    if (PV.M > 0)
        k_schur_obs_rs<<<nblk(PV.M, 64), 64, 0, s>>>(PV, Mr, nloc, vobs, vcoff, J, Lb, W);
}
void launch_schur_init(hipStream_t s, const DevProblem &P, const double *Acc, const double *Acg,
                       const double *Agg, const double *g, const double *diag, double lam,
                       const SView &V, int npad, double *rhs, const RedSpec *red,
                       const double *partial, double *scalar) {
    const int n = P.ncf * PCMAX + P.nG + npad;
    if (red && red->nrows > 0)
        k_schur_init_red<<<nblk(n, 256) + red->nrows, 256, 0, s>>>(
            P, Acc, Acg, Agg, g, diag, lam, V, npad, rhs, nblk(n, 256), partial, *red, scalar);
    else
        k_schur_init<<<nblk(n, 256), 256, 0, s>>>(P, Acc, Acg, Agg, g, diag, lam, V, npad, rhs);
    if (P.rs) launch_rs_offdiag(s, P, V);
    if (P.ls_ng > 0) launch_lens_shared_offdiag(s, P, V);
}
void launch_schur_pairs(hipStream_t s, const DevProblem &P, const double *W, const double *Wg,
                        const double *tb, const SView &V, double *rhs) {
    if (P.nB == 0) return;
    k_schur_pairs<<<nblk(P.nB, 64), 64, 0, s>>>(P, W, Wg, tb, V, rhs);
}
bool launch_schur_dest(hipStream_t s, const DevProblem &P, const double *W, const int2 *dest,
                       const int *dest_off, int ndest, const int2 *pairs, const SView &V,
                       int pc_uniform, int assign_off, const double *tb, double *rhs,
                       SchurInitFold fold, const int *wave_list, int n_wave,
                       const int *lane_list, int n_lane) {
    if (ndest <= 0) return false;
    const int nw = lane_list ? n_wave : ndest;
    const int *wl = lane_list ? wave_list : nullptr;
    const int lg = 8 * ((nblk(n_lane, 256) + 7) / 8);
    if (pc_uniform == 6) {
        if (nw > 0)
            k_schur_dest_u<6><<<8 * ((nw + 7) / 8), 64, 0, s>>>(P, W, dest, dest_off, pairs, V,
                                                                assign_off, nw, tb, rhs, fold, wl);
        if (lane_list)
            k_schur_dest_lane<6><<<lg, 256, 0, s>>>(P, W, dest, dest_off, pairs, V, assign_off,
                                                    lane_list, n_lane);
        return rhs != nullptr;
    }
    if (pc_uniform == 7) {
        if (nw > 0)
            k_schur_dest_u<7><<<8 * ((nw + 7) / 8), 64, 0, s>>>(P, W, dest, dest_off, pairs, V,
                                                                assign_off, nw, tb, rhs, fold, wl);
        if (lane_list)
            k_schur_dest_lane<7><<<lg, 256, 0, s>>>(P, W, dest, dest_off, pairs, V, assign_off,
                                                    lane_list, n_lane);
        return rhs != nullptr;
    }
    k_schur_dest<<<ndest, 64, 0, s>>>(P, W, dest, dest_off, pairs, V, assign_off);
    return false;
}
void launch_schur_rhs(hipStream_t s, const DevProblem &P, const double *W, const double *tb,
                      double *rhs) {
    if (P.ncf > 0) k_schur_rhs<<<P.ncf, 64, 0, s>>>(P, W, tb, rhs);
}
void launch_schur_glob(hipStream_t s, const DevProblem &P, const double *W, const double *Wg,
                       const double *tb, const SView &V, double *rhs) {
    if (P.nG > 0 && P.nB > 0)
        k_schur_glob<<<nblk(P.nB, 64), 64, 0, s>>>(P, W, Wg, tb, V, rhs);
}
void launch_backsub_bundle(hipStream_t s, const DevProblem &P, const double *W, const double *Wg,
                           const double *tb, const double *Lb, const double *xR, double *U,
                           double *x) {
    if (P.nB == 0) return;
    constexpr bool two_pass = true;
    if (two_pass) {
        k_obs_wtx<<<nblk(P.M, 64), 64, sizeof(double) * 64 * P.wst, s>>>(P, W, xR, U);
        k_backsub_bundle<<<nblk(P.nB, 64), 64, 0, s>>>(P, nullptr, U, Wg, tb, Lb, xR, x);
    } else {
        k_backsub_bundle<<<nblk(P.nB, 64), 64, 0, s>>>(P, W, nullptr, Wg, tb, Lb, xR, x);
    }
}
void launch_scatter_xR(hipStream_t s, const DevProblem &P, const double *xR, double *x) {
    k_scatter_xR<<<nblk(P.n, 256), 256, 0, s>>>(P, xR, x);
}
void launch_newton_bundle(hipStream_t s, const DevProblem &P, const double *W, const double *Wg,
                          const double *Lb, const double *v, double *wR, double *usq,
                          double *un, double *gp) {
// ... 61 lines not shown
```

mayamatchmovesolver_amd/csrc/mmba_lm.cpp:

```cpp
#include <algorithm>
#include <cfloat>
#include <chrono>
#include <thread>
#include <cmath>
#include <cstdio>
#include <cstring>

#include "mmba_geom.h"
#include "mmba_kernels.h"
#include "mmba_plan.h"

namespace mmba {

constexpr bool kBacksubGroup = true;
constexpr bool kBacksubGroupOnepass = true;

static double wall_now() {
    return std::chrono::duration<double>(std::chrono::steady_clock::now().time_since_epoch())
        .count();
}

hipEvent_t Plan::next_event() {
    if (ev_used == ev_pool.size()) {
        hipEvent_t e = nullptr;
// ... 128 lines not shown
    }
    if (!mirrored)
        MMBA_HIP(hipMemcpyAsync(h_scalar + lo, d_scalar + lo, sizeof(double) * (hi - lo + 1),
                                hipMemcpyDeviceToHost, s));
    if (nranks > 1 && comm && comm->bounded()) {
        host_sync();
        return;
    }
    if (!ev_sync) MMBA_HIP(hipEventCreateWithFlags(&ev_sync, hipEventDisableTiming));
    MMBA_HIP(hipEventRecord(ev_sync, s));
    for (;;) {
        const hipError_t e = hipEventQuery(ev_sync);
        if (e == hipSuccess) break;
        if (e != hipErrorNotReady) MMBA_HIP(e);
    }
}

void Plan::stream_wait() {
    if (!ev_sync) MMBA_HIP(hipEventCreateWithFlags(&ev_sync, hipEventDisableTiming));
    MMBA_HIP(hipEventRecord(ev_sync, s));
    wait_event();
}

double Plan::read_scalar(int slot) {
    read_slots(slot, slot);
    return h_scalar[slot];
}

void Plan::allreduce(double *d, size_t count, ReduceOp op) {
    if (comm && nranks > 1) comm->allreduce(d, count, op, s);
}

double Plan::reduce_read(int slot, ReduceOp op) {
    allreduce(d_scalar + slot, 1, op);
    return read_scalar(slot);
}

void Plan::dnorm_enqueue(const double *dv, int slot) {
    launch_sumsq(s, dv, d_diag, n, d_partial, nparts, d_scalar + slot, d_p_own, d_ticket);
    allreduce(d_scalar + slot, 1);
}

double Plan::dnorm(const double *dv) {
    dnorm_enqueue(dv, SL_DNORM);
    return std::sqrt(read_scalar(SL_DNORM));
}

void Plan::records_enqueue(const double *xat, int base_only) {
    launch_records(s, P, d_var_cf, d_ext_pert, d_step, d_recs, nvar, d_brec, base_only, &orec);
    recs_full_at = base_only ? nullptr : xat;
}

void Plan::fun_enqueue(const double *dx, double *df, double *eu, double *ed, double *dist,
                       int slot) {
    flush_red();
    launch_param_set(s, P, dx, d_ext, d_ext_pert, d_step, opt.solver_type, opt.delta, fd_eps());
    params_at = dx;
    records_enqueue(dx, 0);
    span_begin(SPAN_RESID);
    launch_rows_eval(s, P, df + 2 * (size_t)M, eu ? eu + 2 * (size_t)M : nullptr, d_partial,
                     (M + 255) / 256);
    launch_residual(s, P, d_recs, df, eu, ed, d_partial, d_scalar + slot,
                    P.nrows > 0 ? nullptr : d_ticket, dist, &orec);
    span_end(SPAN_RESID);
    allreduce(d_scalar + slot, 1);
}

double Plan::fun(const double *dx, double *df, double *eu, double *ed, double *dist) {
    const double t0 = wall_now();
    fun_enqueue(dx, df, eu, ed, dist);
    const double r = std::sqrt(read_scalar(SL_FNORM));
    t_func += wall_now() - t0;
    return r;
}

bool Plan::pre_jac_ok() const {
    return pre_jac && nranks == 1 && !central && nrows == 0 && !timing && ne_epilogue_fusable(P) &&
           jac_ne_fusable(P, jac_ncv) && !(cbk && cbk->interrupt) && !(cbk && cbk->progress);
}

bool Plan::trial_red_fold() const {
    const int pin = path_choice(MMBA_PATH_TRIAL_RED_FOLD);
    return pin < 0 ? kTrialRedFold : pin != 0;
}

NeEpi Plan::fused_epi(const double *dx, const JacLM &lm) const {
    NeEpi e;
    e.on = 1;
    e.first = lm.first;
    e.mode = lm.mode;
    e.fnorm = lm.fnorm;
    e.fnorm_sq = lm.fnorm_sq;
    e.do_xn = lm.first;
    e.do_gn = lm.fnorm_sq || lm.fnorm != 0.;
    e.x = dx;
    e.diag = d_diag;
    e.acnorm = d_acnorm;
    e.partial = d_partial;
    e.rstride = pw;
    e.cf_base = 0;
    e.bnd_base = ncf;
    e.probe = d_k2probe;
    return e;
}

static bool epi_lb0(const Plan &pl, NeEpi &e) {
    if (!(pl.P.nbs > 0 && pl.P.JB != nullptr && pl.nB_solved > 0)) return false;
    e.Lb = pl.d_Lb;
    e.tb = pl.d_tb;
    e.fail = pl.d_fail;
    return true;
}

static void epi_jb(const Plan &pl, NeEpi &e) {
    if (!pl.jb_recompute()) return;
    e.jb_recs = pl.d_recs;
    e.jb_lmder = pl.opt.solver_type == MMBA_SOLVER_CMINPACK_LMDER ? 1 : 0;
}

static void epi_cf_split(const Plan &pl, NeEpi &e) {
    if (path_choice(MMBA_PATH_NE_CF_SPLIT) == 0) return;
    e.cf_part = pl.d_cf_part;
    e.cf_ticket = pl.d_cf_ticket;
}

static int epi_ncol(const Plan &pl) {
    return pl.ncf + (pl.nB_solved > 0 ? (pl.nB + NE_BND_TPB - 1) / NE_BND_TPB : 0);
}

static RedSpec epi_rows(int pw, int ncol, int do_xn, int do_gn, int s_zero = Plan::SL_ZERO,
                        int s_xn2 = Plan::SL_XN2, int s_gnorm = Plan::SL_GNORM) {
    RedSpec rs{};
    rs.flag_slot = -1;
    rs.row[rs.nrows++] = {0, ncol, 1, s_zero};
    if (do_xn) rs.row[rs.nrows++] = {pw, ncol, 0, s_xn2};
    if (do_gn) rs.row[rs.nrows++] = {2 * pw, ncol, 1, s_gnorm};
    return rs;
}

void Plan::epi_reduce(int ncol, int do_xn, int do_gn) {
    if (nranks > 1) {
        double *tail = d_Agg + NGMAX * NGMAX + NGMAX;
        MMBA_HIP(hipMemsetAsync(tail, 0, sizeof(double) * (2 + nranks), s));
        launch_reduce_multi(s, d_partial, epi_rows(pw, ncol, do_xn, do_gn, 0, 1, 2 + rank), tail);
        allreduce(tail, 2 + nranks);
        launch_fold_ranks(s, tail, nranks, d_scalar + SL_ZERO, do_xn, do_gn);
        return;
    }
    const RedSpec rs = epi_rows(pw, ncol, do_xn, do_gn);
    if (fl.sobs_ahead) {
    } else if (red_defer_ok() && !timing) {
        pend_rs = rs;
        fl.pend_red = true;
    } else {
        launch_reduce_multi(s, d_partial, rs, d_scalar);
    }
}

void Plan::pre_jac_enqueue(const double *dx, double *eu, double *ed, const TrialRed &red) {
    const JacLM lm{0, opt.auto_param_scale == 1 ? 1 : 2, 0., d_scalar + SL_FNORM};
    NeEpi epi = fused_epi(dx, lm);
    epi.gate = d_gate;
    launch_jac_ne(s, jb_recompute() ? P_nojb() : P, d_recs, d_step, opt.solver_type, d_J, d_jcol,
                  nloc_set ? nullptr : d_nloc, d_stale, eu, ed, d_Acc, d_g, epi, red);
    nloc_set = true;
    fl.pre_jac_pending = true;
    fl.pre_bnd_pending = false;
    bool lb0 = false;
    if (P.nbs > 0 && P.JB != nullptr && nG == 0) {
        epi_jb(*this, epi);
        lb0 = epi_lb0(*this, epi);
        launch_ne(s, P, d_J, d_jcol, d_nloc, d_f, d_Acc, d_Acg, d_Abb, d_Abg, d_Agg, d_g,
                  d_glob_partial, glob_chunk, epi, true);
        fl.pre_bnd_pending = true;
    }
    fl.pre_sobs_pending = false;
    if (fl.pre_bnd_pending && lb0 && !rs_bnd && red_defer_ok() &&
        path_choice(MMBA_PATH_PRE_SCHUR) == 1) {
        const RedSpec rs = epi_rows(pw, epi_ncol(*this), epi.do_xn, epi.do_gn);
        launch_schur_obs(s, P, d_J, d_Lb, d_W, &rs, d_partial, d_scalar, d_gate);
        fl.pre_sobs_pending = true;
    }
    fl.pre_jac_x = dx;
}

bool Plan::jb_recompute() const {
    return P.JB != nullptr && P.all_bnd_fast && path_choice(MMBA_PATH_JB_RECOMPUTE) == 1;
}

DevProblem Plan::P_nojb() const {
    DevProblem Q = P;
    Q.JB = nullptr;
    return Q;
}

void Plan::jac(const double *dx, const JacLM *lm) {
    flush_red();
    const double t0 = wall_now();
    const double eps_dif = fd_eps();
    const bool lmder = opt.solver_type == MMBA_SOLVER_CMINPACK_LMDER;
    if (params_at != dx) {
        launch_param_set(s, P, dx, d_ext, d_ext_pert, d_step, opt.solver_type, opt.delta, eps_dif);
        recs_full_at = nullptr;
    }
    params_at = dx;
    if (recs_full_at != dx) records_enqueue(dx, 0);
    CentralB CB;
    if (central) {
        MMBA_HIP(hipMemsetAsync(d_scalar + SL_NCENT, 0, sizeof(double), s));
        launch_param_central(s, P, dx, d_ext_pertB, d_stepB, opt.delta, d_scalar + SL_NCENT,
                             b15 ? d_c15 : nullptr);
        launch_records(s, P, d_var_cf, d_ext_pertB, d_stepB, d_recsB, nvar, d_brecB, 0);
        CB.recs = d_recsB;
        CB.brec = d_brecB;
        CB.ext_pert = d_ext_pertB;
        CB.step = d_stepB;
        if (b15) {
            launch_b15_q(s, P, d_c15, d_q15, d_kap15, d_c15r);
            CB.q15 = d_q15;
            CB.kap15 = d_kap15;
        }
    }
    span_begin(SPAN_JAC);
    const bool fuse = lm && ne_epilogue_fusable(P) && nrows == 0 && !b15;
    NeEpi epi;
    epi.probe = d_k2probe;
    fl.lb0_valid = false;
    if (fuse) {
        epi = fused_epi(dx, *lm);
        epi_cf_split(*this, epi);
        fl.lb0_valid = epi_lb0(*this, epi);
    }
    const bool k2_fused = !central && jac_ne_fusable(P, jac_ncv);
    const bool pre_done = fl.pre_jac_pending && fl.pre_jac_x == dx && k2_fused && fuse;
    if (nranks > 1) MMBA_HIP(hipMemsetAsync(d_g, 0, sizeof(double) * n, s));
    fl.pre_jac_pending = false;
    const bool pre_bnd = pre_done && fl.pre_bnd_pending;
    fl.pre_bnd_pending = false;
    fl.sobs_ahead = pre_done && fl.pre_sobs_pending;
    fl.pre_sobs_pending = false;
    if (pre_done) {
    } else if (k2_fused) {
        launch_jac_ne(s, jb_recompute() ? P_nojb() : P, d_recs, d_step, opt.solver_type, d_J,
                      d_jcol, nloc_set ? nullptr : d_nloc, d_stale, d_eu, d_ed, d_Acc, d_g, epi);
        nloc_set = true;
    } else {
        launch_jacobian(s, P, d_recs, d_ext_pert, d_step, opt.solver_type, d_J, d_jcol, d_nloc,
                        d_stale, d_eu, d_ed, jac_ncv, d_f, CB, &orec);
    }
    if (k2_fused) epi_jb(*this, epi);
    launch_rows_jac(s, P, d_ext, d_ext_pert, d_step, central ? d_ext_pertB : nullptr,
                    central ? d_stepB : nullptr, lmder ? 1 : 0, d_Jrow, d_eu + 2 * (size_t)M,
                    n - 1);
    if (!pre_bnd &&
        launch_ne(s, P, d_J, d_jcol, d_nloc, d_f, d_Acc, d_Acg, d_Abb, d_Abg, d_Agg, d_g,
                  d_glob_partial, glob_chunk, epi, k2_fused))
        ++ne_split_launches;
    launch_rows_ne(s, P, d_Jrow, d_f + 2 * (size_t)M, d_p_own, d_Acc, d_Abb, d_Agg, d_g);
    if (nG > 0) allreduce(d_Agg, NGMAX * NGMAX + NGMAX);
    if (fuse) {
        span_end(SPAN_JAC);
        epi_reduce(epi_ncol(*this), epi.do_xn, epi.do_gn);
    } else if (!lm) {
        launch_colnorms(s, P, d_Acc, d_Abb, d_Agg, d_acnorm, d_g);
        span_end(SPAN_JAC);
    } else {
        const int do_xn = lm->first, do_gn = lm->fnorm_sq || lm->fnorm != 0.;
        if (b15) {
            launch_b15_s(s, lm->fnorm_sq, lm->fnorm, d_b15k + 4);
            launch_b15_unrot(s, P, d_Acc, d_g, d_q15, d_adiag15, d_u15);
        }
        launch_jac_epilogue(s, P, d_Acc, d_Abb, d_Agg, d_acnorm, d_g, d_diag, dx, lm->first,
                            lm->mode, lm->fnorm, lm->fnorm_sq, do_xn, do_gn, d_p_own, d_partial,
                            nparts, pw, b15 ? d_c15 : nullptr, d_b15k + 4, d_g15, d_adiag15,
                            d_u15);
        span_end(SPAN_JAC);
        epi_reduce(nparts, do_xn, do_gn);
    }
    t_jac += wall_now() - t0;
}

static TrialFold trial_fold_base(const Plan &pl) {
    TrialFold T;
    T.x = pl.d_x;
    T.diag = pl.d_diag;
    T.wa1 = pl.d_wa1;
    T.wa2 = pl.d_wa2;
    T.wa3 = pl.d_wa3;
    T.ext = pl.d_ext;
    T.ext_pert = pl.d_ext_pert;
    T.step = pl.d_step;
    T.solver_type = pl.opt.solver_type;
    T.delta = pl.opt.delta;
    T.eps_dif = pl.fd_eps();
    T.partial = pl.d_partial + 3 * (size_t)pl.pw;
    T.rstride = pl.pw;
    T.own = pl.d_p_own;
    T.recs = pl.d_recs;
    T.brec = pl.d_brec;
    return T;
}

void Plan::trial_enqueue(double *eu, double *ed, bool with_dnorm, bool fill_dnorm,
                         const LmDec *dec, bool jac_ahead) {
    flush_red();
    const double t0 = wall_now();
    double *pr = d_partial + 3 * (size_t)pw;
    const int tparts = trial_folded     ? trial_fold_parts(P, n_trial_other, trial_rec)
                       : trial_prep_rec ? trial_prep_rec_parts(P, n_prep_other)
// ... 64 lines not shown
        fl.seq_pending = true;
        ++trial_red_folds;
    } else {
        if (mirror) ++seq_next;
        launch_reduce_multi(s, d_partial, rs, d_scalar, flag, mirror ? h_scalar : nullptr,
                            SL_LAST + 1, d_mticket, mirror ? h_seq : nullptr, seq_next, D);
        fl.seq_pending = mirror;
    }
    if (b15)
        launch_b15_jp(s, n, d_xs15r, d_g, d_c15r, d_b15k + 4, d_scalar + SL_JP);
    fl.mirror_pending = mirror;
    fl.pre_hb_enq = hb_enq;
    if (fl.pre_hb_enq)
        MMBA_HIP(hipEventRecord(ev_hb[3], s));
    if (dec && jac_ahead) {
        stage_slots();
        pre_jac_enqueue(d_wa2, eu, ed, R);
    }
    if (fl.pre_hb_enq) {
        MMBA_HIP(hipStreamWaitEvent(s_hb[0], ev_hb[3], 0));
        launch_handback_host(s_hb[0], Mg, nrows, d_dev_of_ref, d_f, eu, ed, pre_hb_map[0],
                             pre_hb_map[1], pre_hb_map[2], d_scalar + SL_DGO, d_ftrial);
        hb_used[0] = true;
        hb_pending = true;
    }
    allreduce(d_scalar + SL_PNORM, with_dnorm ? 6 : 4);
    t_func += wall_now() - t0;
}

void Plan::solve_damped_enqueue(double lam, int dnorm_slot, bool defer, bool dnorm_by_trial) {
    if (nranks > 1 && path_choice(MMBA_PATH_FAULT_SHARD) == rank + 1)
        throw Invalid{"injected shard fault (MMBA_PATH_FAULT_SHARD)"};
    if (nranks > 1 && path_choice(MMBA_PATH_STALL_SHARD) == rank + 1 && !stall_done) {
        stall_done = true;
        std::this_thread::sleep_for(std::chrono::milliseconds(2 * (long long)comm_timeout_ms()));
    }
    if (!red_defer_ok()) flush_red();
    fl.fail_early = false;
    if (b15 && !b15_inner) {
        b15_inner = true;
        launch_b15_accl(s, P, d_Acc, d_q15, d_diag, lam, d_AccL, d_diagL);
        std::swap(d_Acc, d_AccL);
        std::swap(d_diag, d_diagL);
        solve_damped_enqueue(lam, -1, false, false);
        MMBA_HIP(hipMemcpyAsync(d_z15u, d_xs, sizeof(double) * n, hipMemcpyDeviceToDevice, s));
        MMBA_HIP(hipMemcpyAsync(d_b15k + 5, d_scalar + SL_FAIL, sizeof(double),
                                hipMemcpyDeviceToDevice, s));
        std::swap(d_g, d_c15r);
        solve_damped_enqueue(lam, -1, false, false);
        std::swap(d_g, d_c15r);
        std::swap(d_Acc, d_AccL);
        std::swap(d_diag, d_diagL);
        MMBA_HIP(hipMemcpyAsync(d_z15c, d_xs, sizeof(double) * n, hipMemcpyDeviceToDevice, s));
        b15_inner = false;
        launch_b15_combine(s, n, d_g, d_c15r, d_z15u, d_z15c, d_b15k + 4, d_xs15r, d_b15k,
                           d_scalar, SL_FAIL, d_b15k + 5);
        launch_b15_rot(s, P, d_q15, d_xs15r, d_xs);
        if (dnorm_slot >= 0) launch_b15_dnorm(s, n, d_xs, d_diag, d_scalar + dnorm_slot);
        (void)defer;
        (void)dnorm_by_trial;
        return;
    }
    const double t0 = wall_now();
    trial_folded = false;
    if (bd_one_launch() && dnorm_slot >= 0) {
        span_begin(SPAN_CHOL);
        bd_direct(s, P, bs.bd, d_Acc, d_g, d_diag, lam, d_xR, d_xs, d_fail, d_scalar, dnorm_slot,
                  SL_FAIL, fl.pend_red ? &pend_rs : nullptr, d_partial);
        fl.pend_red = false;
        span_end(SPAN_CHOL);
        t_linear += wall_now() - t0;
        return;
    }
    if (nB_solved > 0) {
        if (!(lam == 0. && fl.lb0_valid))
            launch_bundle_factor(s, P, d_Abb, d_Abg, d_g, d_diag, lam, d_Lb, d_tb, d_Wg, d_fail);
        const bool ahead = fl.sobs_ahead && lam == 0. && fl.lb0_valid && !rs_bnd;
        fl.sobs_ahead = false;
        fl.lb0_valid = false;
        if (rs_bnd)
            launch_schur_obs_rs(s, PV, M, d_nloc, d_vobs, d_vcoff, d_J, d_Lb, d_W);
        else if (!ahead) {
            launch_schur_obs(s, P, d_J, d_Lb, d_W, fl.pend_red ? &pend_rs : nullptr, d_partial,
                             d_scalar);
            fl.pend_red = false;
        }
    }
    const DevProblem &PS = schur_problem();
    if (nR > 0) {
        const Reduced kind = reduced_now();
        const SView V = sview();
        if (nranks > 1) MMBA_HIP(hipMemsetAsync(d_rhs, 0, sizeof(double) * nRpad, s));
        if (band && bs.red) {
            MMBA_HIP(hipMemsetAsync(bs.red, 0, sizeof(double) * (bs.red_count - nRpad), s));
        } else if (band && ((!bs.use_bcr && kind != Reduced::BlockDiag) || rs_bnd || lens_shared)) {
            const int nb = nR - nG;
            MMBA_HIP(hipMemsetAsync(bs.Bd, 0, sizeof(double) * (size_t)nb * (bw + 1), s));
            if (nG > 0) MMBA_HIP(hipMemsetAsync(bs.Ga, 0, sizeof(double) * (size_t)nG * nb, s));
            MMBA_HIP(hipMemsetAsync(bs.Gd, 0, sizeof(double) * NGMAX * NGMAX, s));
        } else if (kind == Reduced::Dense) {
            MMBA_HIP(hipMemsetAsync(d_S, 0, sizeof(double) * (size_t)(nRpad + 1) * dld, s));
        } else if (!band) {
            MMBA_HIP(hipMemsetAsync(d_S, 0, sizeof(double) * (size_t)nslots * TILE * TILE, s));
        }
        const bool fold = fold_init && nB_solved > 0;
        if (!fold) {
            launch_schur_init(s, P, d_Acc, d_Acg, d_Agg, d_g, d_diag, lam, V, nRpad - nR, d_rhs,
                              fl.pend_red ? &pend_rs : nullptr, d_partial, d_scalar);
            fl.pend_red = false;
        }
        flush_red();
        if (nB_solved > 0) {
            if (use_dest) {
                SchurInitFold fi{};
                if (fold) fi = SchurInitFold{1, d_Acc, d_g, d_diag, lam};
                const bool rhs_done =
                    launch_schur_dest(s, PS, d_W, d_dest, d_dest_off, ndest, d_dpairs, V,
                                      pc_uniform, band && bs.use_bcr && !rs_bnd, d_tb, d_rhs, fi,
                                      d_dest_wave, n_dest_wave, d_dest_lane, n_dest_lane);
                if (!rhs_done) launch_schur_rhs(s, PS, d_W, d_tb, d_rhs);
                launch_schur_glob(s, PS, d_W, d_Wg, d_tb, V, d_rhs);
            } else {
                launch_schur_pairs(s, PS, d_W, d_Wg, d_tb, V, d_rhs);
            }
        }
        if (dbg_keep_S && dense) {
            MMBA_HIP(hipMemcpyAsync(d_Skeep, ds.A, sizeof(double) * (size_t)ds.ld * (ds.n + 1),
                                    hipMemcpyDeviceToDevice, s));
            MMBA_HIP(hipMemcpyAsync(d_rkeep, d_rhs, sizeof(double) * nRpad, hipMemcpyDeviceToDevice,
                                    s));
        }
        span_begin(SPAN_CHOL);
        switch (kind) {
        case Reduced::BlockDiag:
            bd_factor_solve(s, bs.bd, d_fail, d_rhs, d_yR, d_xR, d_xs);
            break;
        case Reduced::Pcr:
            if (bs.red) allreduce(bs.red, bs.red_count);
            pcr_solve(s, bs.pcr, d_rhs, d_xR, bs.pcr.row_param ? d_xs : nullptr, d_fail);
            break;
        case Reduced::Band:
            if (bs.red) allreduce(bs.red, bs.red_count);
            band_factor_forward(s, bs, d_fail, d_probe, d_rhs, d_yR);
            break;
        case Reduced::Dense:
            if (nranks > 1) {
                allreduce(d_S, (size_t)ds.ld * (ds.n + 1));
                allreduce(d_rhs, nRpad);
            }
            ds.factor_forward(s, d_rhs, d_yR, d_fail);
            break;
        case Reduced::TiledNarrow:
        case Reduced::Tiled:
            for (int k = 0; k < NT; ++k) {
                const int r0 = panel_rows_off[k], nr = panel_rows_off[k + 1] - r0;
                launch_chol_panel(s, d_S, d_slot, NT, k, d_rows + r0, nr, d_Linv, d_fail);
                const int q0 = panel_pairs_off[k], nq = panel_pairs_off[k + 1] - q0;
                launch_chol_update(s, d_S, d_slot, NT, k, d_pairs + q0, nq);
            }
            break;
        }
        span_end(SPAN_CHOL);
        bool scattered = false;
        switch (kind) {
        case Reduced::BlockDiag:
            scattered = true;
            break;
// ... 976 lines not shown
```

mayamatchmovesolver_amd/csrc/mmba_plan.cpp:

```cpp
#include <algorithm>
#include <climits>
#include <cmath>
#include <cstdio>
#include <cstdlib>
#include <cstring>
#include <map>
#include <unordered_map>
#include <numeric>
#include <set>

#include "mmba_kernels.h"
#include "mmba_plan.h"

namespace mmba {

Plan::~Plan() {
    if (d_k2probe) {
        std::vector<long long> t(5 * (size_t)ncf);
        if (hipMemcpy(t.data(), d_k2probe, sizeof(long long) * t.size(), hipMemcpyDeviceToHost) ==
            hipSuccess) {
            long long t0 = LLONG_MAX, tend = 0;
            for (int c = 0; c < ncf; ++c)
                if (t[5 * c]) {
                    t0 = std::min(t0, t[5 * c]);
                    tend = std::max(tend, t[5 * c + 3]);
                }
            std::vector<double> st, stg, obs, tail, tot;
            int per_xcc[16] = {};
            for (int c = 0; c < ncf; ++c) {
                const long long *q = &t[5 * c];
                if (!q[0]) continue;
                st.push_back((q[0] - t0) / 100.);
                stg.push_back((q[1] - q[0]) / 100.);
                obs.push_back((q[2] - q[1]) / 100.);
                tail.push_back((q[3] - q[2]) / 100.);
                tot.push_back((q[3] - q[0]) / 100.);
                per_xcc[q[4] & 15]++;
            }
            auto pct = [](std::vector<double> v, double p) {
                if (v.empty()) return 0.;
                std::sort(v.begin(), v.end());
                return v[std::min(v.size() - 1, (size_t)(p * (v.size() - 1) + 0.5))];
            };
            std::fprintf(stderr, "[mmba probe] k_jac_ne_u %zu workgroups, span %.2f us; p0/p50/p100 "
                                 "(us): start %.2f/%.2f/%.2f staging %.2f/%.2f/%.2f observations "
                                 "%.2f/%.2f/%.2f tail %.2f/%.2f/%.2f total %.2f/%.2f/%.2f; per XCC",
                         st.size(), (tend - t0) / 100., pct(st, 0), pct(st, .5), pct(st, 1),
                         pct(stg, 0), pct(stg, .5), pct(stg, 1), pct(obs, 0), pct(obs, .5),
                         pct(obs, 1), pct(tail, 0), pct(tail, .5), pct(tail, 1), pct(tot, 0),
                         pct(tot, .5), pct(tot, 1));
            for (int x = 0; x < 8; ++x) std::fprintf(stderr, " %d", per_xcc[x]);
            std::fprintf(stderr, "\n");
        }
    }
    if (d_probe && bs.use_bcr && bs.bcr.fflags && bs.bcr.nblk >= 2) {
        const int nit = bs.bcr.nblk + 64;
        std::vector<long long> t((size_t)8 + 4 * nit, 0);
        if (hipMemcpy(t.data(), d_probe, sizeof(long long) * t.size(), hipMemcpyDeviceToHost) ==
            hipSuccess) {
            std::fprintf(stderr,
                         "[mmba probe] bcr df phase 10-ns ticks (workgroup 0, all items, all solves): "
                         "stage %lld a-load %lld chain %lld store %lld mfma-upd %lld tail %lld\n",
                         t[0], t[1], t[2], t[3], t[4], t[5]);
            const long long *tr = t.data() + 8;
            long long t0 = tr[0];
            for (int i = 0; i < nit && (tr[4 * i] || tr[4 * i + 3]); ++i) t0 = std::min(t0, tr[4 * i]);
            int base = 0, lvl = 0;
            for (int nact = bs.bcr.nblk;; nact = (nact + 1) / 2, ++lvl) {
                const int g = nact > 1 ? (nact + 1) / 2 : 1;
                double w = 0, c = 0, p = 0, lo = 1e30, hi = 0;
                for (int i = base; i < base + g; ++i) {
                    const long long *q = tr + 4 * i;
                    w += q[1] - q[0];
                    c += q[2] - q[1];
                    p += q[3] - q[2];
                    lo = std::min(lo, (double)(q[1] - t0));
                    hi = std::max(hi, (double)(q[3] - t0));
                }
                std::fprintf(stderr,
                             "[mmba probe] bcr df level %d items %d: wait %.2f item %.2f publish "
                             "%.2f us (means); work from %.2f to %.2f us\n",
                             lvl, g, w / g / 100., c / g / 100., p / g / 100., lo / 100.,
                             hi / 100.);
                base += g;
                if (nact <= 1) break;
            }
        }
    } else if (d_probe && bs.use_bcr) {
        long long h[6] = {0, 0, 0, 0, 0, 0};
        if (hipMemcpy(h, d_probe, sizeof(h), hipMemcpyDeviceToHost) == hipSuccess)
            std::fprintf(stderr,
                         "[mmba probe] bcr level 10-ns ticks (workgroup 0, all levels): stage %lld "
                         "a-load %lld chain %lld store %lld mfma-upd %lld tail %lld (K=%d nblk=%d)\n",
                         h[0], h[1], h[2], h[3], h[4], h[5], bs.bcr.K, bs.bcr.nblk);
    } else if (d_probe) {
        long long h[4] = {0, 0, 0, 0};
        if (hipMemcpy(h, d_probe, sizeof(h), hipMemcpyDeviceToHost) == hipSuccess)
            std::fprintf(stderr,
                         "[mmba probe] band factor cycles (partition 0): diag+move %lld panel %lld "
                         "update %lld tail %lld (nb=%d w=%d nG=%d P=%d)\n",
                         h[0], h[1], h[2], h[3], nR - nG, bw, nG, bs.P);
    }
    for (hipEvent_t e : ev_pool) (void)hipEventDestroy(e);
    if (ev_sync) (void)hipEventDestroy(ev_sync);
    if (hb_pending)
        for (hipStream_t c : s_hb)
            if (c) (void)hipStreamSynchronize(c);
    for (hipEvent_t e : ev_hb)
        if (e) (void)hipEventDestroy(e);
    for (hipStream_t c : s_hb)
        if (c) (void)hipStreamDestroy(c);
    for (void *p : allocs) (void)hipFree(p);
    if (h_scalar) (void)hipHostFree(h_scalar);
    if (h_fail) (void)hipHostFree(h_fail);
    if (h_bflag) (void)hipHostFree(h_bflag);
    if (h_xstage) (void)hipHostFree(h_xstage);
    if (h_seq) (void)hipHostFree(h_seq);
    if (h_pack) (void)hipHostFree(h_pack);
    if (h_met) (void)hipHostFree(h_met);
}

static void require(bool c, const char *what) {
    if (!c) throw Invalid{what};
}

void shard_layout(int F, int M, const int32_t *obs_frame, const int32_t *obs_bnd, int nB,
                  int nranks, int32_t *bounds, int32_t *bnd_owner) {
    std::vector<long long> per_frame(F + 1, 0);
    for (int i = 0; i < M; ++i) per_frame[obs_frame[i] + 1]++;
    for (int f = 0; f < F; ++f) per_frame[f + 1] += per_frame[f];
    for (int k = 0; k <= nranks; ++k) bounds[k] = F;
    bounds[0] = 0;
    for (int k = 1; k < nranks; ++k) {
        const long long target = (long long)k * M / nranks;
        int f = bounds[k - 1];
// ... 1119 lines not shown
    D.cf_frame = upload(cf_frame);
    D.cf_obs_off = upload(cf_obs_off);
    D.cf_var_off = upload(cf_var_off);
    D.cf_var_param = upload(cf_var_param);
    D.cf_var_flags = upload(cf_var_flags);
    D.cf_pc = upload(cf_pc);
    D.cf_roff = upload(cf_roff);
    D.pc_uniform = pc_uniform;
    D.wst = 3 * (pc_uniform > 0 ? pc_uniform : PCMAX);
    D.bnd_par_off = upload(bnd_par_off);
    D.bnd_par = upload(bnd_par);
    D.bnd_pb = upload(bnd_pb);
    D.bnd_xoff = nullptr;
    D.bnd_p4 = upload(bnd_p4);
    {
        bool ok = true;
        for (int c = 0; c < nC && ok && !rs_on; ++c)
            if (pr->tfm_parent[pr->cam_tfm[c]] >= 0) ok = false;
        D.cf_aidx = nullptr;
        if (ok && ncf > 0) {
            static const int cam_k[7] = {MMBA_CAM_FILM_BACK_W_INCH, MMBA_CAM_FILM_BACK_H_INCH,
                                         MMBA_CAM_FILM_OFFSET_X_INCH, MMBA_CAM_FILM_OFFSET_Y_INCH,
                                         MMBA_CAM_FOCAL_MM, MMBA_CAM_FAR_CLIP, MMBA_CAM_SCALE};
            std::vector<int> tab((size_t)CF_AIDX * ncf, -1);
            auto vidx = [&](int a, int f) -> int {
                if (a < 0) return -1;
                const long long ix = pr->attr_offset[a] + (pr->attr_animated[a] ? f : 0);
                if (ix > INT32_MAX) throw Unsupported{"attribute block over 2^31 values"};
                return (int)ix;
            };
            for (int cf = 0; cf < ncf; ++cf) {
                const int c = cf_cam[cf], f = cf_frame[cf];
                for (int k = 0; k < 7; ++k)
                    tab[(size_t)CF_AIDX * cf + k] =
                        vidx(pr->cam_attrs[MMBA_CAM_NUM_ATTRS * c + cam_k[k]], f);
                const int t = pr->cam_tfm[c];
                for (int k = 0; k < 9; ++k)
                    tab[(size_t)CF_AIDX * cf + 7 + k] = vidx(pr->tfm_attrs[9 * t + k], f);
            }
            D.cf_aidx = upload(tab);
        }
    }
    D.nbs = nB_solved;
    D.dest_diag_ii = dest_diag_ii ? 1 : 0;
    D.all_bnd_fast = 1;
    for (int b = 0; b < nB; ++b)
        if (bnd_p4[b].w < 0) D.all_bnd_fast = 0;
    D.no_lens = 1;
    for (int c = 0; c < nC; ++c)
        if (pr->cam_lens && pr->cam_lens[c] >= 0) D.no_lens = 0;
    {
        std::vector<int> bpos(M);
        for (int q = 0; q < M; ++q) bpos[bobs[q]] = q;
        D.obs_bpos = upload(bpos);
        bool all_fast = nG == 0 && nB_solved > 0 && !rs_on;
        for (int b = 0; b < nB && all_fast; ++b)
            if (bnd_pb[b] > 0 && bnd_p4[b].w < 0) all_fast = false;
        D.JB = all_fast ? dalloc<double>((size_t)8 * M) : nullptr;
        bool fast = nG == 0 && (pc_uniform == 6 || pc_uniform == 7);
        for (int b = 0; b < nB && fast; ++b)
            if (bnd_pb[b] > 0 && bnd_p4[b].w < 0) fast = false;
        for (int c = 0; c < nC && fast; ++c)
            if (pr->cam_lens && pr->cam_lens[c] >= 0) fast = false;
        for (size_t t = 0; t < cf_var_flags.size() && fast; ++t)
            if (cf_var_flags[t] != 0) fast = false;
        for (int cf = 0; cf < ncf && fast; ++cf)
            if (cf_var_off[cf + 1] - cf_var_off[cf] - 1 > pc_uniform) fast = false;
        if (central || opt.robust_loss || rs_on) fast = false;
        jac_ncv = fast ? pc_uniform : 0;
        D.jcol_implicit = jac_ncv > 0 ? 1 : 0;
    }
    d_brec = dalloc<double>((size_t)nB * BREC);
    D.brec = d_brec;
    D.bobs_off = upload(bobs_off);
    D.bobs = upload(bobs);
    {
        std::vector<int2> rp(M);
        for (int q = 0; q < M; ++q) {
            const int cf = d_cf[bobs[q]];
            rp[q] = make_int2(cf_roff[cf], cf_pc[cf]);
        }
        d_bobs_rp = upload(rp);
    }
    D.cam_lpar_off = upload(cam_lpar_off);
    {
        bool any_inst = false;
        for (int i = 0; i < M; ++i) any_inst |= d_inst[i] >= 0;
        if (any_inst) {
            D.obs_inst = upload(d_inst);
            D.inst_lens = upload(inst_lens_h);
            D.inst_attr = upload(inst_attr_h);
            D.inst_frame = upload(inst_frame_h);
            D.inst_val = upload(inst_val_h);
            D.inst_lpar_off = upload(inst_lpar_off_h);
            D.inst_lpar = upload(inst_lpar_h.empty() ? std::vector<int>{-1} : inst_lpar_h);
            d_inst_attr_plug = upload(std::vector<int>(inst_attr_h.size(), -1));
        } else {
            D.obs_inst = nullptr;
        }
    }
    D.cam_lpar = upload(cam_lpar);
    {
        int lm = 1;
        for (int i = 0; i < M; ++i) lm = std::max(lm, obs_cols(i));
        D.lmax = std::min(lm, LMAX);
    }
    D.p_attr = upload(pr->param_attr, n);
    D.p_frame = upload(pr->param_frame, n);
    D.p_class = upload(p_class);
    D.p_pos = upload(p_pos);
    D.p_both = upload(p_both);
    D.p_blk = upload(p_blk);
    D.p_min = upload(pr->param_min, n);
    D.p_max = upload(pr->param_max, n);
    D.p_off = upload(pr->param_offset, n);
    D.p_scale = upload(pr->param_scale, n);
    D.g_param = upload(g_param);
    D.root = rank == 0 ? 1 : 0;
    D.Ra = Ra;
    D.Rb = Rb;
    D.nrows = nrows;
    D.rows_live = opt.scene_graph_mode == MMBA_SCENE_GRAPH_MM_SCENE_GRAPH ? 0 : 1;
    D.row_attr = upload(row_attr);
    D.row_frame = upload(row_frame);
    D.row_param = upload(row_param);
    D.row_w = upload(row_w);
    D.row_var = upload(row_var);
    D.row_val = upload(row_val);
    D.p_vidx = upload(param_vidx);
    D.bnd_vx = nullptr;
    D.bnd_pcomp = nullptr;
    {
        bool ok = nB > 0;
        bool fwd = true;
        std::vector<int4> vx(std::max(nB, 1), make_int4(-1, -1, -1, 0));
        std::vector<int> pcomp(std::max(nB, 1), 0);
        for (int b = 0; b < nB && ok; ++b) {
            const int t = pr->bnd_tfm[b];
            if (pr->tfm_parent[t] >= 0) {
                ok = false;
                break;
            }
            int ix[3];
            for (int k = 0; k < 3; ++k) {
                const int a = pr->tfm_attrs[9 * t + k];
                if (a >= 0 && pr->attr_animated[a]) ok = false;
                const long long v = a < 0 ? -1 : (long long)pr->attr_offset[a];
                if (v > INT32_MAX) ok = false;
                ix[k] = (int)v;
            }
            vx[b] = make_int4(ix[0], ix[1], ix[2], 0);
            const int4 p4 = bnd_p4[b];
            if (p4.w < 0) continue;
            const int ps[3] = {p4.x, p4.y, p4.z};
            int seen = 0;
            for (int a = 0; a < p4.w && ok; ++a) {
                const int pa = pr->param_attr[ps[a]];
                int comp = -1;
                for (int k = 0; k < 3; ++k)
                    if (pr->tfm_attrs[9 * t + k] == pa) comp = k;
                if (comp < 0) {
                    ok = false;
                } else {
                    pcomp[b] |= comp << (2 * a);
                    if ((seen >> comp) & 1 || param_vidx[ps[a]] != (long long)ix[comp])
                        fwd = false;
// ... 181 lines not shown
    p_class_h = p_class;
    p_blk_h = p_blk;
    P = D;
    if (rs_bnd) {
        PV = P;
        PV.M = Mv;
        PV.obs_cf = upload(v_cf);
        PV.obs_bnd = upload(v_bnd);
        PV.cf_obs_off = upload(vcf_off);
        PV.bobs_off = upload(vbobs_off);
        PV.bobs = upload(vbobs);
        d_vobs = upload(v_obs);
        d_vcoff = upload(v_coff);
    }

    d_var_cf = upload(var_cf);
    d_stale = upload(stale);
    d_ref_of_dev = upload(ref_of_dev);
    {
        std::vector<int> dev_of_own(Mg, -1);
        for (int i = 0; i < M; ++i)
            if (obs_own_g[ref_of_dev[i]]) dev_of_own[ref_of_dev[i]] = i;
        setup_metrics(F, nK, Mg, pr->obs_marker, pr->obs_frame, dev_of_own);
    }
    if (nranks == 1 && M > 0) {
        std::vector<int> dev_of_ref(M, 0);
        for (int i = 0; i < M; ++i) dev_of_ref[ref_of_dev[i]] = i;
        d_dev_of_ref = upload(dev_of_ref);
    }
    d_slot = upload(slot);
    d_rows = upload(panel_rows);
    d_cols = upload(panel_cols);
    d_pairs = upload(pairs);
    d_rows_off = upload(panel_rows_off);
    d_cols_off = upload(panel_cols_off);
    if (use_dest) {
        d_dest = upload(dest_h);
        d_dest_off = upload(dest_off_h);
        d_dpairs = upload(dpairs_h);
        if (pc_uniform == 6 || pc_uniform == 7) {
            std::vector<int> wl, ll;
            for (int d = 0; d < ndest; ++d) {
                const bool lane = dest_h[d].x != dest_h[d].y && dest_off_h[d + 1] - dest_off_h[d] <= 32;
                (lane ? ll : wl).push_back(d);
            }
            const int pin = path_choice(MMBA_PATH_DEST_LANE);
            if (!ll.empty() && pin != 0 &&
                (pin == 1 || (ll.size() >= 16384 && 2 * ll.size() >= (size_t)ndest))) {
                n_dest_wave = (int)wl.size();
                n_dest_lane = (int)ll.size();
                d_dest_wave = upload(wl.empty() ? std::vector<int>(1, 0) : wl);
                d_dest_lane = upload(ll);
            }
        }
    }
    {
        const long long full = (long long)NT * (NT + 1) / 2;
        dense = !band && nranks == 1 && NT >= 8 && (long long)nslots * 10 >= full * 3;
        if (path_choice(MMBA_PATH_DENSE) >= 0)
            dense = !band && nranks == 1 && NT > 0 && path_choice(MMBA_PATH_DENSE) != 0;
        if (shard_dense) dense = true;
    }
    if (dense) {
        ds.setup(*this, nRpad);
        d_S = ds.A;
        dld = ds.ld;
        d_Linv = nullptr;
        if (nranks > 1) d_ymask = upload(std::vector<int>(std::max(nR, 1), rank == 0 ? 1 : 0));
    } else {
        d_S = dalloc<double>((size_t)nslots * TILE * TILE);
        d_Linv = dalloc<double>((size_t)NT * TILE * TILE);
    }
    cfblk_roff.clear();
    cfblk_pc.clear();
    cfblk_cf.clear();
    for (int cf = 0; cf < ncf; ++cf)
        if (cf_pc[cf] > 0) {
            cfblk_roff.push_back(cf_roff[cf]);
            cfblk_pc.push_back(cf_pc[cf]);
            cfblk_cf.push_back(cf);
        }
    if (band) setup_band();
    if (path_choice(MMBA_PATH_PROBE) == 2) {
        d_k2probe = dalloc<long long>(5 * (size_t)std::max(ncf, 1));
        MMBA_HIP(hipMemsetAsync(d_k2probe, 0, 5 * (size_t)std::max(ncf, 1) * sizeof(long long), s));
    }
    if (band && path_choice(MMBA_PATH_PROBE) == 1) {
        const size_t np = 8 + 4 * ((size_t)std::max(nR, 1) + 64);
        d_probe = dalloc<long long>(np);
        MMBA_HIP(hipMemsetAsync(d_probe, 0, np * sizeof(long long), s));
    }

    d_x = dalloc<double>(n);
    d_ext = dalloc<double>(n);
    d_ext_pert = dalloc<double>(n);
    d_step = dalloc<double>(n);
    d_diag = dalloc<double>(n);
    d_acnorm = dalloc<double>(n);
    d_g = dalloc<double>(n);
    d_wa1 = dalloc<double>(n);
    d_wa2 = dalloc<double>(n);
    d_wa3 = dalloc<double>(n);
    d_xs = dalloc<double>(n);
    d_v = dalloc<double>(n);
    d_f = dalloc<double>(m);
    d_ftrial = dalloc<double>(m);
    d_eu = dalloc<double>(m);
    d_ed = dalloc<double>(M);
    d_eu_s = dalloc<double>(m);
    d_ed_s = dalloc<double>(M);
    for (double *b : {d_f, d_ftrial, d_eu, d_eu_s})
        MMBA_HIP(hipMemsetAsync(b, 0, sizeof(double) * m, s));
    d_Jrow = dalloc<double>(nrows);
    d_dist_x = dalloc<double>(M);
    d_dist_t = dalloc<double>(M);
    d_recs = dalloc<double>((size_t)nvar * CAMREC);
    if (central) {
        d_ext_pertB = dalloc<double>(n);
        d_stepB = dalloc<double>(n);
        d_recsB = dalloc<double>((size_t)nvar * CAMREC);
        d_brecB = dalloc<double>((size_t)nB * BREC);
    }
    if (b15) {
        d_c15 = dalloc<double>(n);
        d_c15r = dalloc<double>(n);
        d_g15 = dalloc<double>(n);
        d_z15u = dalloc<double>(n);
        d_z15c = dalloc<double>(n);
        d_q15 = dalloc<double>((size_t)ncf * PCMAX * PCMAX);
        d_kap15 = dalloc<double>(ncf);
        d_AccL = dalloc<double>((size_t)ncf * PCMAX * PCMAX);
        d_diagL = dalloc<double>(n);
        d_xs15r = dalloc<double>(n);
        d_p15 = dalloc<double>(n);
        d_v15 = dalloc<double>(n);
        d_adiag15 = dalloc<double>(n);
        d_u15 = dalloc<double>(n);
        d_b15k = dalloc<double>(8);
        MMBA_HIP(hipMemsetAsync(d_b15k, 0, sizeof(double) * 8, s));
    }
    d_J = dalloc<double>(std::max((size_t)2 * D.lmax * M, (size_t)m + M));
    d_jcol = dalloc<int>((size_t)std::max(D.lmax, 1) * M);
    d_nloc = dalloc<int>(M);
    d_Acc = dalloc<double>((size_t)ncf * PCMAX * PCMAX);
    d_cf_part = dalloc<double>((size_t)std::max(ncf, 1) * NE_CF_SPLIT * NE_CF_NT);
    d_cf_ticket = dalloc<unsigned>((size_t)std::max(ncf, 1));
    MMBA_HIP(hipMemsetAsync(d_cf_ticket, 0, sizeof(unsigned) * std::max(ncf, 1), s));
    d_Acg = dalloc<double>((size_t)ncf * PCMAX * NGMAX);
    d_Abb = dalloc<double>((size_t)nB * 9);
    d_Abg = dalloc<double>((size_t)nB * PBMAX * NGMAX);
    d_Agg = dalloc<double>(NGMAX * NGMAX + NGMAX + 2 + std::max(nranks, 1));
    d_gather = dalloc<double>((size_t)2 * mg + Mg + n);
    if (nranks > 1) setup_handback(obs_rank_g);
    d_glob_partial = dalloc<double>((size_t)((M + glob_chunk - 1) / glob_chunk) * (NGMAX * NGMAX + NGMAX));
    d_Lb = dalloc<double>((size_t)nB * 9);
    d_tb = dalloc<double>((size_t)nB * 3);
    d_Wg = dalloc<double>((size_t)nB * NGMAX * 3);
    const int Mw = rs_bnd ? std::max(Mv, 1) : M;
    d_W = dalloc<double>((size_t)P.wst * (nB_solved > 0 ? Mw : 1));
    d_U = dalloc<double>((size_t)4 * (nB_solved > 0 ? Mw : 1));
    d_rhs = bs.red_rhs ? bs.red_rhs : dalloc<double>(nRpad);
    d_yR = dalloc<double>(nRpad);
    d_xR = dalloc<double>(nRpad);
    d_wR = dalloc<double>(nRpad);
    d_usq = dalloc<double>(nB);
    d_nu = dalloc<double>((size_t)3 * std::max(nB, 1));
    d_ngp = dalloc<double>((size_t)std::max(nG, 1) * std::max(nB, 1));
    pw = std::max(std::max(nparts, residual_blocks(P)), ncf + (nB + NE_BND_TPB - 1) / NE_BND_TPB);
// ... 463 lines not shown
```

mayamatchmovesolver_amd/csrc/mmba_plan.h:

```cpp
#pragma once

#include <hip/hip_runtime.h>

#include <algorithm>
#include <cfloat>
#include <cmath>
#include <memory>
#include <string>
#include <vector>

#include "mmba_internal.h"
#include "mmba_kernels.h"

struct mmba_context {
    int device = 0;
    hipStream_t stream = nullptr;
    std::vector<mmba_context *> shards;
    std::vector<mmba::Comm *> comms;
};

namespace mmba {

void set_error(const std::string &msg);
int path_choice(int key);
// ... 259 lines not shown
    } fl;
    enum class Reduced { BlockDiag, Pcr, Band, Dense, TiledNarrow, Tiled };
    Reduced reduced_now() const;
    bool bd_one_launch() const;
    bool sep_pcr_now() const;
    bool dataflow_off();

    enum Slot {
        SL_PNORM = 0,
        SL_XN2T = 1,
        SL_FNORM = 2,
        SL_JP = 3,
        SL_DNORM = 4,
        SL_FAIL = 5,
        SL_NEWT_B = 6,
        SL_NEWT_R = 7,
        SL_GDIV = 8,
        SL_ZERO = 9,
        SL_XN2 = 10,
        SL_GNORM = 11,
        SL_RMS = 12,
        SL_NCENT = 13,
        SL_F0 = 14,
        SL_DGO = 15,
        SL_DRATIO = 16,
        SL_DDELTA = 17,
        SL_DPAR = 18,
        SL_DINFO = 19,
        SL_LAST = 19,
        SL_FI = 20,
        SL_ESUM = 21,
        SL_ENMIN = 22,
        SL_EMAX = 23,
        SL_IESUM = 24,
        SL_IENMIN = 25,
        SL_IEMAX = 26,
        NSLOT = 28
    };
    void read_slots(int lo, int hi);
    hipEvent_t ev_sync = nullptr;
    double read_scalar(int slot = 0);
    void stream_wait();
    void allreduce(double *d, size_t count, ReduceOp op = ReduceOp::Sum);
    double reduce_read(int slot, ReduceOp op = ReduceOp::Sum);
    void fun_enqueue(const double *dx, double *df, double *eu, double *ed,
                     double *dist = nullptr, int slot = SL_FNORM);
    double fun(const double *dx, double *df, double *eu, double *ed, double *dist = nullptr);
    double *d_dist_x = nullptr, *d_dist_t = nullptr;
    std::vector<long long> param_vidx;
    std::vector<double> pmin_h, pmax_h, poff_h, pscale_h;
    void error_stats_device(const double *ed, double *avg, double *mn, double *mx);
    void error_stats_enqueue(const double *ed, int base = SL_ESUM);
    struct JacLM {
        int first, mode;
        double fnorm;
        const double *fnorm_sq = nullptr;
    };
    void jac(const double *dx, const JacLM *lm = nullptr);
    NeEpi fused_epi(const double *dx, const JacLM &lm) const;
    void epi_reduce(int ncol, int do_xn, int do_gn);
    const mmba_callbacks *cbk = nullptr;
    bool poll_interrupt() const {
        return cbk && cbk->interrupt && cbk->interrupt(cbk->user) != 0;
    }
    void jac_partial_stale(const double *dx, int k);
    void trial_enqueue(double *eu, double *ed, bool with_dnorm = false, bool fill_dnorm = false,
                       const LmDec *dec = nullptr, bool jac_ahead = false);
    bool trial_fold_ok = false, trial_folded = false;
    bool trial_rec = false;
    int2 *d_bobs_rp = nullptr;
    bool brec_fwd = false;
    bool trial_prep_rec = false;
    int *d_prep_other = nullptr;
    int n_prep_other = 0;
    int *d_trial_other = nullptr;
    int n_trial_other = 0;
    bool pre_jac = true;
    int *d_gate = nullptr;
    bool pre_jac_ok() const;
    void pre_jac_enqueue(const double *dx, double *eu, double *ed,
                         const TrialRed &red = TrialRed());
    static constexpr bool kTrialRedFold = true;
    bool trial_red_fold() const;
    void stage_slots();
    RedSpec pend_rs{};
    bool red_defer_ok() const;
    void flush_red();
    void host_sync();
    bool jb_recompute() const;
    DevProblem P_nojb() const;
    bool stall_done = false;
    double *d_cf_part = nullptr;
    unsigned *d_cf_ticket = nullptr;
    void wait_event();
    double *d_eu_s = nullptr, *d_ed_s = nullptr;
    bool spec_ok = true;
    bool outputs_ready = false;
    const double *params_at = nullptr;
    const double *recs_full_at = nullptr;
    void records_enqueue(const double *xat, int base_only);
    void attrs_reset() {
        MMBA_HIP(hipMemcpyAsync(P.attr_val, d_attr0, attr_bytes, hipMemcpyDeviceToDevice, s));
        params_at = nullptr;
        recs_full_at = nullptr;
    }
    double fd_eps() const { return std::sqrt(std::max(std::fabs(opt.delta), DBL_EPSILON)); }
    int pw = 0;
    void solve_damped_enqueue(double lam, int dnorm_slot = -1, bool defer = false,
                              bool dnorm_by_trial = false);
    bool solve_damped(double lam);
    void newton_enqueue(double dxnorm);
    void dnorm_enqueue(const double *dv, int slot);
    double dnorm(const double *dv);
    int solve(double *x_inout, double *fvec_out, double *eu_out, double *ed_out,
              mmba_result *res, const mmba_callbacks *cb, mmba_trace *trace);
    int solve_once(double *x_inout, double *fvec_out, double *eu_out, double *ed_out,
                   mmba_result *res, const mmba_callbacks *cb, mmba_trace *trace);
    int spec_replays = 0;
    bool batch_ok = false;
    std::string batch_why;
    int batch_nf = 0, batch_nfmax = 0;
    int *d_fr_cf_off = nullptr, *d_fr_par_off = nullptr, *d_fr_par = nullptr,
        *d_fr_last = nullptr, *d_fr_nobs = nullptr;
    double *d_bJ = nullptr, *d_bdist = nullptr, *d_bx = nullptr, *d_bpw = nullptr;
    BatchOut *d_bout = nullptr;
    int *h_bflag = nullptr, *d_bflag = nullptr;
    int solve_frames(double *x_inout, mmba_result *results, const mmba_callbacks *cb);
    int dense_jacobian(const double *x, double *fjac);
    bool dbg_keep_S = false;
    double *d_Skeep = nullptr, *d_rkeep = nullptr;
    int reduced_residual(const double *x, double lam, double *relres);
    bool dbg_jcol_stored = false;
    double *d_dbg_flag = nullptr;
    double *d_dbg_pack = nullptr;
    void handback_step(double *step_out, double *g_out, double *diag_out);
    void assemble_dense_jacobian(double *fjac, bool own_rows = false);
    int damped_step(const double *x, double lam, double *step_out, double *g_out,
                    double *diag_out, double *fjac_out);
    int reproject(const double *x, double *point_out, double *marker_out);
    int measure(const double *x, double *fvec_out, double *eu_out, double *ed_out,
                double *stats);
    void download_params(const double *dx, double *x_out);
    void download_ref_order(const double *d_f2, const double *d_eu2, const double *d_ed1,
                            double *f_out, double *eu_out, double *ed_out, bool sync = true);
    hipStream_t s_hb[3] = {nullptr, nullptr, nullptr};
    hipEvent_t ev_hb[4] = {nullptr, nullptr, nullptr, nullptr};
    bool hb_pending = false;
    bool hb_used[3] = {false, false, false};
    void handback_wait();
    void handback_streams();
    bool map_outputs(double *f_out, double *eu_out, double *ed_out, double *hmap[3]);
    bool pre_hb_on = false;
    long long pre_handbacks = 0;
    long long ne_split_launches = 0;
    long long trial_red_folds = 0;
    double *pre_hb_map[3] = {nullptr, nullptr, nullptr};
    MetricsDev met{};
    int met_F = 0, met_K = 0;
    double *d_met_coll = nullptr;
    char *h_met = nullptr;
    void setup_metrics(int F, int K, int Mg, const int32_t *obs_marker, const int32_t *obs_frame,
                       const std::vector<int> &dev_of_own);
    void error_metrics(mmba_error_metrics *out);
};

}
// ... 37 lines not shown
```

mayamatchmovesolver_amd/csrc/mmba_wave_dev.h:

```cpp
#pragma once

#include <hip/hip_runtime.h>

namespace mmba {

__device__ __forceinline__ double wave_rsq(double d) {
    double y = __builtin_amdgcn_rsq(d);
    const double h = 0.5 * d;
    y = y * fma(-h * y, y, 1.5);
    y = y * fma(-h * y, y, 1.5);
    return y;
}

__device__ __forceinline__ double wave_rdlane(double v, int l) {
    const long long x = __double_as_longlong(v);
    const int lo = __builtin_amdgcn_readlane((int)(x & 0xffffffffll), l);
    const int hi = __builtin_amdgcn_readlane((int)(x >> 32), l);
    return __longlong_as_double(((long long)hi << 32) | (unsigned int)lo);
}

__device__ __forceinline__ void wave_lds_sync() {
    __builtin_amdgcn_fence(__ATOMIC_SEQ_CST, "wavefront");
    __builtin_amdgcn_wave_barrier();
}

typedef __attribute__((address_space(1))) unsigned int gu32_t;
typedef __attribute__((address_space(1))) unsigned long long gu64_t;

__device__ __forceinline__ void st_sc1(double *p, double v) {
    __hip_atomic_store((gu64_t *)p, (unsigned long long)__double_as_longlong(v), __ATOMIC_RELAXED,
                       __HIP_MEMORY_SCOPE_AGENT);
}

__device__ __forceinline__ double ld_sc1(const double *p) {
    return __longlong_as_double((long long)__hip_atomic_load(
        (gu64_t *)const_cast<double *>(p), __ATOMIC_RELAXED, __HIP_MEMORY_SCOPE_AGENT));
}

__device__ __forceinline__ __amdgpu_buffer_rsrc_t sc1_view(const double *base, unsigned bytes) {
    return __builtin_amdgcn_make_buffer_rsrc(const_cast<double *>(base), 0, bytes, 0x00020000);
}
__device__ __forceinline__ double sc1_load(__amdgpu_buffer_rsrc_t r, int idx) {
    return __builtin_bit_cast(double, __builtin_amdgcn_raw_buffer_load_b64(r, idx * 8, 0, 16));
}

__device__ __forceinline__ double wave_sum(double v) {
#pragma unroll
    for (int off = 32; off > 0; off >>= 1) v += __shfl_xor(v, off);
    return v;
}
__device__ __forceinline__ double wave_max(double v) {
#pragma unroll
    for (int off = 32; off > 0; off >>= 1) v = fmax(v, __shfl_xor(v, off));
    return v;
}

__device__ __forceinline__ void block_tree(double *red, bool mx = false) {
    for (int w = 128; w > 0; w >>= 1) {
        if (threadIdx.x < w)
            red[threadIdx.x] = mx ? fmax(red[threadIdx.x], red[threadIdx.x + w])
                                  : red[threadIdx.x] + red[threadIdx.x + w];
        __syncthreads();
    }
}

template <int N>
__device__ __forceinline__ void wave_chol_aug(double (&a)[N], double &rsl, bool &bad) {
    const int lane = threadIdx.x & 63;
#pragma unroll
    for (int j = 0; j < N; ++j) {
        double d = wave_rdlane(a[j], j);
        if (!(d > 0.) || !isfinite(d)) {
            bad = true;
            d = 1.;
        }
        const double rs = wave_rsq(d);
        const double l = (lane > j) ? a[j] * rs : 0.;
        a[j] = (lane == j) ? d * rs : (lane > j ? l : a[j]);
        if (lane == j) rsl = rs;
#pragma unroll
        for (int c = j + 1; c < N; ++c) a[c] = fma(-l, wave_rdlane(l, c), a[c]);
    }
}

}
```

Measured before the change: 2.135 billion residuals/s.

## Hoist epilogue loads ahead of barriers and pack per-observation Schur metadata

Adds a default-on loads_first path. In the Jacobian and normal-equation kernel, diag, x and fnorm values are loaded before the first barrier and staged in shared memory. Parameter indices are read from shared memory, and the wave reduction uses permlane swaps plus DPP moves instead of shuffles. The bundle kernel preloads its epilogue operands before the observation loop, and k_schur_obs reads a packed per-observation int (start slot, pc, pb) instead of chasing obs_cf, cf_pc and cf_var_off. The aim is to cut dependent global-load latency in the tails, at the cost of extra shared memory, a new device array, and probe instrumentation.

Result: faster. 2.198 billion residuals/s, median of 6 (+3.0%).

```diff
diff --git a/include/mmba.h b/include/mmba.h
--- a/include/mmba.h
+++ b/include/mmba.h
@@ -332,7 +332,8 @@
 #define MMBA_PATH_OBJ_CF 27
 #define MMBA_PATH_OBJ_REC 28
 #define MMBA_PATH_PCR_WIDE 29
-#define MMBA_PATH_NUM 30
+#define MMBA_PATH_LOADS_FIRST 30
+#define MMBA_PATH_NUM 31
 int mmba_debug_set_path(int key, int value);
 
 int mmba_debug_band_solve(mmba_context *ctx, int nb, int w, int nG, int P, const double *S,
diff --git a/mayamatchmovesolver_amd/abi.py b/mayamatchmovesolver_amd/abi.py
--- a/mayamatchmovesolver_amd/abi.py
+++ b/mayamatchmovesolver_amd/abi.py
@@ -48,7 +48,8 @@
 PATH_OBJ_CF = 27
 PATH_OBJ_REC = 28
 PATH_PCR_WIDE = 29
-PATH_NUM = 30
+PATH_LOADS_FIRST = 30
+PATH_NUM = 31
 
 FILM_FIT_FILL = 0
 FILM_FIT_HORIZONTAL = 1
diff --git a/mayamatchmovesolver_amd/csrc/mmba_api.cpp b/mayamatchmovesolver_amd/csrc/mmba_api.cpp
--- a/mayamatchmovesolver_amd/csrc/mmba_api.cpp
+++ b/mayamatchmovesolver_amd/csrc/mmba_api.cpp
@@ -12,10 +12,10 @@
 static thread_local std::string g_last_error;
 void set_error(const std::string &msg) { g_last_error = msg; }
 
-static_assert(MMBA_PATH_NUM == 30, "one initialiser per path key");
+static_assert(MMBA_PATH_NUM == 31, "one initialiser per path key");
 static std::atomic<int> g_path[MMBA_PATH_NUM] = {-1, -1, -1, -1, -1, -1, -1, -1, -1, -1, -1, -1, -1,
                                                  -1, -1, -1, -1, -1, -1, -1, -1, -1, -1, -1, -1,
-                                                 -1, -1, -1, -1, -1};
+                                                 -1, -1, -1, -1, -1, -1};
 int path_choice(int key) {
     return (key > 0 && key < MMBA_PATH_NUM) ? g_path[key].load() : -1;
 }
diff --git a/mayamatchmovesolver_amd/csrc/mmba_internal.h b/mayamatchmovesolver_amd/csrc/mmba_internal.h
--- a/mayamatchmovesolver_amd/csrc/mmba_internal.h
+++ b/mayamatchmovesolver_amd/csrc/mmba_internal.h
@@ -206,6 +206,7 @@
     int no_lens;
     const int *obs_bpos;
     double *JB;
+    const int *obs_sp;
     const int *cam_lpar_off, *cam_lpar;
     const int *obs_inst, *inst_lens, *inst_attr, *inst_frame, *inst_lpar_off, *inst_lpar;
     const double *inst_val;
diff --git a/mayamatchmovesolver_amd/csrc/mmba_kernels.h b/mayamatchmovesolver_amd/csrc/mmba_kernels.h
--- a/mayamatchmovesolver_amd/csrc/mmba_kernels.h
+++ b/mayamatchmovesolver_amd/csrc/mmba_kernels.h
@@ -127,7 +127,9 @@
     int *fail = nullptr;
     const int *gate = nullptr;
     long long *probe = nullptr;
-};
+    int loads_first = 0;
+};
+constexpr int K2_PROBE_N = 8;
 struct TrialRed {
     int on = 0;
     RedSpec spec{};
@@ -156,7 +158,7 @@
                           double *Lb, double *tb, double *Wg, int *fail);
 void launch_schur_obs(hipStream_t s, const DevProblem &P, const double *J, const double *Lb,
                       double *W, const RedSpec *red = nullptr, const double *partial = nullptr,
-                      double *scalar = nullptr, const int *gate = nullptr);
+                      double *scalar = nullptr, const int *gate = nullptr, bool packed = false);
 void launch_schur_obs_rs(hipStream_t s, const DevProblem &PV, int Mr, const int *nloc,
                          const int *vobs, const int *vcoff, const double *J, const double *Lb,
                          double *W);
diff --git a/mayamatchmovesolver_amd/csrc/mmba_kernels.hip b/mayamatchmovesolver_amd/csrc/mmba_kernels.hip
--- a/mayamatchmovesolver_amd/csrc/mmba_kernels.hip
+++ b/mayamatchmovesolver_amd/csrc/mmba_kernels.hip
@@ -705,8 +705,8 @@
     if (E.do_gn) q.fn = own ? sqrt(fsq_own) : E.fnorm_sq ? sqrt(*E.fnorm_sq) : E.fnorm;
     return q;
 }
-__device__ __forceinline__ void epi_param_pre(const NeEpi &E, const EpiPre &q, double d, double gp,
-                                              double &zf, double &xn, double &gm) {
+__device__ __forceinline__ double epi_param_pre(const NeEpi &E, const EpiPre &q, double d,
+                                                double gp, double &zf, double &xn, double &gm) {
     const double an = sqrt(d);
     E.acnorm[q.p] = an;
     double dg = q.dg;
@@ -723,6 +723,7 @@
     if (E.do_gn && an != 0.) {
         if (q.fn != 0.) gm = fmax(gm, fabs((gp / q.fn) / an));
     }
+    return dg;
 }
 template <int PC>
 __device__ __forceinline__ void epi_params_wave(const DevProblem &P, const NeEpi &E, int cf,
@@ -1026,7 +1027,7 @@
     return lm_decide_vals(R.dec, tin);
 }
 
-template <int PC, int NW, bool GEN>
+template <int PC, int NW, bool GEN, bool LF>
 __global__ void __launch_bounds__(64 * NW) k_jac_ne_u(
     DevProblem P, const double *__restrict__ recs, const double *__restrict__ step,
     int solver_type, double *__restrict__ J, int *__restrict__ jcol, int *__restrict__ nloc,
@@ -1039,6 +1040,7 @@
     __shared__ double sSt[PC];
     __shared__ int sHdr[3];
     __shared__ double sTr[5];
+    __shared__ double sDg[LF ? PC : 1], sXv[LF ? PC : 1], sFs[1];
     if (!R.on && E.gate &&
         __hip_atomic_load(E.gate, __ATOMIC_RELAXED, __HIP_MEMORY_SCOPE_AGENT) == 0)
         return;
@@ -1058,11 +1060,12 @@
         return;
     }
     const int cf = xcd_remap((int)blockIdx.x - pad, ncf);
-    long long *pr = (E.probe && threadIdx.x == 0) ? E.probe + 5 * (size_t)cf : nullptr;
+    long long *pr = (E.probe && threadIdx.x == 0) ? E.probe + K2_PROBE_N * (size_t)cf : nullptr;
     const long long t_in = pr ? (long long)wall_clock64() : 0;
     const int o0 = P.cf_obs_off[cf], o1 = P.cf_obs_off[cf + 1];
     const bool lmder = solver_type == MMBA_SOLVER_CMINPACK_LMDER;
     const bool solved = P.cf_pc[cf] == PC && own_cf(P, cf);
+    [[maybe_unused]] int pE = -1;
     {
         constexpr int KT = ((PC + 1) * CAMREC + 64 * NW - 1) / (64 * NW);
         const int voff = P.cf_var_off[cf];
@@ -1077,6 +1080,7 @@
         const int fr = P.cf_frame[cf];
         if (R.on) trial_rows_issue<NW>(R, tin, TR);
         const double stv = p >= 0 ? step[p] : 1.;
+        pE = p;
 #pragma unroll
         for (int k = 0; k < KT; ++k) {
             const int t = tid + 64 * NW * k;
@@ -1093,8 +1097,25 @@
         }
     }
     if (R.on) trial_rows_finish<NW>(R, sTr, TR);
+    [[maybe_unused]] double dgv = 0., xvv = 0., fsv = 0.;
+    if constexpr (LF) {
+        if (E.on) {
+            if (pE >= 0) {
+                dgv = E.diag[pE];
+                xvv = E.x[pE];
+            }
+            if (tid == 0 && !R.on && E.fnorm_sq) fsv = *E.fnorm_sq;
+        }
+    }
     __syncthreads();
     if (R.on && trial_decide(R, sTr, tin, TR.dn_dup).go == 0) return;
+    if constexpr (LF) {
+        if (tid < PC) {
+            sDg[tid] = dgv;
+            sXv[tid] = xvv;
+        }
+        if (tid == 0) sFs[0] = fsv;
+    }
     if (pr) {
         pr[0] = t_in;
         pr[1] = (long long)wall_clock64();
@@ -1135,11 +1156,16 @@
 #pragma unroll
     for (int e = 0; e < NE; ++e) {
         double v = acc[e];
-#pragma unroll
-        for (int off = 32; off > 0; off >>= 1) v += __shfl_xor(v, off);
+        if constexpr (LF) {
+            v = wave_sum_lane0(v);
+        } else {
+#pragma unroll
+            for (int off = 32; off > 0; off >>= 1) v += __shfl_xor(v, off);
+        }
         if (lane == 0) wsum[wv][e] = v;
     }
     __syncthreads();
+    if (pr) pr[6] = (long long)wall_clock64();
     double *A = &Acc[(size_t)cf * PCMAX * PCMAX];
     for (int e = tid; e < NE; e += 64 * NW) {
         double v = wsum[0][e];
@@ -1154,10 +1180,13 @@
             const int c = a + rem;
             A[a * PCMAX + c] = v;
             A[c * PCMAX + a] = v;
+        } else if constexpr (LF) {
+            g[sPv[e - NCC]] = v;
         } else {
             g[P.cf_var_param[P.cf_var_off[cf] + 1 + (e - NCC)]] = v;
         }
     }
+    if (pr) pr[7] = (long long)wall_clock64();
     if (E.on && (tid >> 6) == 0) {
         const int ln = tid & 63;
         double d = 0., gp = 0.;
@@ -1171,7 +1200,19 @@
                 gp += wsum[w][NCC + ln];
             }
         }
-        epi_params_wave<PC>(P, E, cf, ln, d, gp, epi_preload<PC>(P, E, cf, ln, R.on != 0, sTr[2]));
+        if constexpr (LF) {
+            EpiPre q{-1, 0., 0., 0.};
+            if (ln < PC) {
+                q.p = sPv[ln];
+                q.dg = sDg[ln];
+                if (E.do_xn) q.xv = sXv[ln];
+                if (E.do_gn) q.fn = R.on ? sqrt(sTr[2]) : E.fnorm_sq ? sqrt(sFs[0]) : E.fnorm;
+            }
+            epi_params_wave<PC>(P, E, cf, ln, d, gp, q);
+        } else {
+            epi_params_wave<PC>(P, E, cf, ln, d, gp,
+                                epi_preload<PC>(P, E, cf, ln, R.on != 0, sTr[2]));
+        }
     }
     if (pr) {
         pr[3] = (long long)wall_clock64();
@@ -1181,6 +1222,7 @@
     }
 }
 
+template <bool LF>
 __global__ void __launch_bounds__(NE_BND_TPB) k_ne_bnd_jb(DevProblem P, double *Abb, double *g,
                                                           NeEpi E) {
     __shared__ double red[3][NE_BND_TPB];
@@ -1195,6 +1237,21 @@
         double gb[PBMAX] = {};
         const int q0 = P.bobs_off[b], q1 = P.bobs_off[b + 1];
         const double *__restrict__ br = &P.brec[(size_t)b * BREC];
+        [[maybe_unused]] EpiPre eq[3] = {{p4.x, 0., 0., 0.}, {p4.y, 0., 0., 0.}, {p4.z, 0., 0., 0.}};
+        if constexpr (LF) {
+            if (E.on) {
+                const double fn =
+                    E.do_gn ? (E.fnorm_sq ? sqrt(*E.fnorm_sq) : E.fnorm) : 0.;
+#pragma unroll
+                for (int a = 0; a < 3; ++a) {
+                    if (a < pb) {
+                        eq[a].dg = E.diag[eq[a].p];
+                        if (E.do_xn) eq[a].xv = E.x[eq[a].p];
+                    }
+                    eq[a].fn = fn;
+                }
+            }
+        }
         for (int qb = q0; qb < q1; qb += 4) {
             double4 u[4], v[4];
             if (E.jb_recs) {
@@ -1254,9 +1311,15 @@
         double dd[3] = {0., 0., 0.};
         if (E.on) {
             double zo = 0., xo = 0., go = 0.;
-            dd[0] = epi_param(E, p4.x, A[0][0], gb[0], zo, xo, go);
-            if (pb > 1) dd[1] = epi_param(E, p4.y, A[1][1], gb[1], zo, xo, go);
-            if (pb > 2) dd[2] = epi_param(E, p4.z, A[2][2], gb[2], zo, xo, go);
+            if constexpr (LF) {
+                dd[0] = epi_param_pre(E, eq[0], A[0][0], gb[0], zo, xo, go);
+                if (pb > 1) dd[1] = epi_param_pre(E, eq[1], A[1][1], gb[1], zo, xo, go);
+                if (pb > 2) dd[2] = epi_param_pre(E, eq[2], A[2][2], gb[2], zo, xo, go);
+            } else {
+                dd[0] = epi_param(E, p4.x, A[0][0], gb[0], zo, xo, go);
+                if (pb > 1) dd[1] = epi_param(E, p4.y, A[1][1], gb[1], zo, xo, go);
+                if (pb > 2) dd[2] = epi_param(E, p4.z, A[2][2], gb[2], zo, xo, go);
+            }
             if (own_bnd(P, b)) {
                 zf = zo;
                 xn = xo;
@@ -1737,7 +1800,7 @@
     }
 }
 
-template <int PCT>
+template <int PCT, bool PK>
 __global__ void __launch_bounds__(64) k_schur_obs(DevProblem P, const double *__restrict__ J,
                                                   const double *__restrict__ Lb, double *W,
                                                   int nob, const RedSpec red,
@@ -1756,20 +1819,42 @@
     const int i = i0 + lane;
     const int M = P.M, wst = P.wst;
     double *row = &sw[lane * wst];
+    int b, pb, pck = 0;
+    if constexpr (PK) {
+        b = i < M ? P.obs_bnd[i] : 0;
+        pck = i < M ? P.obs_sp[i] : 0;
+        pb = pck >> 16;
+    }
     for (int k = 0; k < wst; ++k) row[k] = 0.;
-    const int b = i < M ? P.obs_bnd[i] : 0;
-    const int pb = i < M ? P.bnd_pb[b] : 0;
+    if constexpr (!PK) {
+        b = i < M ? P.obs_bnd[i] : 0;
+        pb = i < M ? P.bnd_pb[b] : 0;
+    }
     if (pb > 0) {
-        const int cf = P.obs_cf[i];
-        const int pc = min(min(P.cf_pc[cf], wst / 3), PCT);
-        const int s = P.cf_var_off[cf + 1] - P.cf_var_off[cf] - 1;
+        int pc, s;
+        if constexpr (PK) {
+            pc = min(min((pck >> 8) & 255, wst / 3), PCT);
+            s = pck & 255;
+        } else {
+            const int cf = P.obs_cf[i];
+            pc = min(min(P.cf_pc[cf], wst / 3), PCT);
+            s = P.cf_var_off[cf + 1] - P.cf_var_off[cf] - 1;
+        }
         double bx[3], by[3], L[3][3], il[3];
+        if constexpr (PK) {
+#pragma unroll
+            for (int a = 0; a < 3; ++a)
+#pragma unroll
+                for (int c = 0; c < 3; ++c) L[a][c] = Lb[(size_t)b * 9 + a * 3 + c];
+        }
 #pragma unroll
         for (int a = 0; a < 3; ++a) {
             bx[a] = a < pb ? J[(size_t)(2 * (s + a)) * M + i] : 0.;
             by[a] = a < pb ? J[(size_t)(2 * (s + a) + 1) * M + i] : 0.;
-#pragma unroll
-            for (int c = 0; c < 3; ++c) L[a][c] = Lb[(size_t)b * 9 + a * 3 + c];
+            if constexpr (!PK) {
+#pragma unroll
+                for (int c = 0; c < 3; ++c) L[a][c] = Lb[(size_t)b * 9 + a * 3 + c];
+            }
         }
 #pragma unroll
         for (int a = 0; a < 3; ++a) il[a] = a < pb ? 1.0 / L[a][a] : 0.;
@@ -3342,19 +3427,20 @@
     const int grid = P.ncf + (R.on ? 8 : 0);
     const long long per = (P.M + P.ncf - 1) / P.ncf;
     int nw = per > 1024 ? 8 : (per > 256 ? 4 : 2);
-#define MMBA_JN(PC, NW, GEN)                                                                  \
-    k_jac_ne_u<PC, NW, GEN><<<grid, 64 * NW, 0, s>>>(P, recs, step, solver_type, J, jcol, nloc, \
-                                                       stale_param, eu, ed, Acc, g, E, R)
-#define MMBA_JN_NW(PC, GEN)                                         \
+#define MMBA_JN_LF(PC, NW, GEN, LF)                                                           \
+    k_jac_ne_u<PC, NW, GEN, LF><<<grid, 64 * NW, 0, s>>>(P, recs, step, solver_type, J, jcol,  \
+                                                           nloc, stale_param, eu, ed, Acc, g, E, R)
+#define MMBA_JN_NW(PC, GEN, LF)                                     \
     do {                                                            \
-        if (nw == 8) MMBA_JN(PC, 8, GEN);                           \
-        else if (nw == 4) MMBA_JN(PC, 4, GEN);                      \
-        else MMBA_JN(PC, 2, GEN);                                   \
+        if (nw == 8) MMBA_JN_LF(PC, 8, GEN, LF);                    \
+        else if (nw == 4) MMBA_JN_LF(PC, 4, GEN, LF);               \
+        else MMBA_JN_LF(PC, 2, GEN, LF);                            \
     } while (0)
 #define MMBA_JN_PC(PC)                                              \
     do {                                                            \
-        if (P.all_bnd_fast) MMBA_JN_NW(PC, false);                  \
-        else MMBA_JN_NW(PC, true);                                  \
+        if (!P.all_bnd_fast) MMBA_JN_NW(PC, true, false);           \
+        else if (E.loads_first) MMBA_JN_NW(PC, false, true);        \
+        else MMBA_JN_NW(PC, false, false);                          \
     } while (0)
     if (P.pc_uniform == 6)
         MMBA_JN_PC(6);
@@ -3362,7 +3448,7 @@
         MMBA_JN_PC(7);
 #undef MMBA_JN_PC
 #undef MMBA_JN_NW
-#undef MMBA_JN
+#undef MMBA_JN_LF
 }
 __global__ void k_fold_ranks(const double *__restrict__ t, int nranks, double *out, int do_xn,
                              int do_gn) {
@@ -3723,8 +3809,10 @@
     }
     if (P.ls_ng > 0) launch_ne_lens_shared(s, P, J, jcol, nloc, f, Acc, Acg, g);
     if (P.nbs > 0) {
-        if (P.JB)
-            k_ne_bnd_jb<<<nblk(P.nB, NE_BND_TPB), NE_BND_TPB, 0, s>>>(P, Abb, g, E);
+        if (P.JB && E.loads_first)
+            k_ne_bnd_jb<true><<<nblk(P.nB, NE_BND_TPB), NE_BND_TPB, 0, s>>>(P, Abb, g, E);
+        else if (P.JB)
+            k_ne_bnd_jb<false><<<nblk(P.nB, NE_BND_TPB), NE_BND_TPB, 0, s>>>(P, Abb, g, E);
         else
             k_ne_bnd<<<nblk(P.nB, 64), 64, 0, s>>>(P, J, jcol, nloc, f, Abb, Abg, g);
     }
@@ -3759,15 +3847,19 @@
 }
 void launch_schur_obs(hipStream_t s, const DevProblem &P, const double *J, const double *Lb,
                       double *W, const RedSpec *red, const double *partial, double *scalar,
-                      const int *gate) {
+                      const int *gate, bool packed) {
     const int nob = nblk(P.M, 64), nr = red ? red->nrows : 0;
     if (nob + nr > 0) {
-        if (P.wst / 3 <= 8)
-            k_schur_obs<8><<<nob + nr, 64, sizeof(double) * 64 * P.wst, s>>>(
-                P, J, Lb, W, nob, red ? *red : RedSpec{}, partial, scalar, gate);
-        else
-            k_schur_obs<PCMAX><<<nob + nr, 64, sizeof(double) * 64 * P.wst, s>>>(
-                P, J, Lb, W, nob, red ? *red : RedSpec{}, partial, scalar, gate);
+#define MMBA_SO(PCT, PK)                                                    \
+    k_schur_obs<PCT, PK><<<nob + nr, 64, sizeof(double) * 64 * P.wst, s>>>( \
+        P, J, Lb, W, nob, red ? *red : RedSpec{}, partial, scalar, gate)
+        const bool pk = packed && P.obs_sp != nullptr;
+        if (P.wst / 3 <= 8) {
+            if (pk) MMBA_SO(8, true); else MMBA_SO(8, false);
+        } else {
+            if (pk) MMBA_SO(PCMAX, true); else MMBA_SO(PCMAX, false);
+        }
+#undef MMBA_SO
     }
 }
 void launch_schur_obs_rs(hipStream_t s, const DevProblem &PV, int Mr, const int *nloc,
diff --git a/mayamatchmovesolver_amd/csrc/mmba_lm.cpp b/mayamatchmovesolver_amd/csrc/mmba_lm.cpp
--- a/mayamatchmovesolver_amd/csrc/mmba_lm.cpp
+++ b/mayamatchmovesolver_amd/csrc/mmba_lm.cpp
@@ -234,6 +234,11 @@
 bool Plan::trial_red_fold() const {
     const int pin = path_choice(MMBA_PATH_TRIAL_RED_FOLD);
     return pin < 0 ? kTrialRedFold : pin != 0;
+}
+
+bool Plan::loads_first() const {
+    const int pin = path_choice(MMBA_PATH_LOADS_FIRST);
+    return pin < 0 ? kLoadsFirst : pin != 0;
 }
 
 NeEpi Plan::fused_epi(const double *dx, const JacLM &lm) const {
@@ -253,6 +258,7 @@
     e.cf_base = 0;
     e.bnd_base = ncf;
     e.probe = d_k2probe;
+    e.loads_first = loads_first() ? 1 : 0;
     return e;
 }
 
@@ -330,7 +336,7 @@
     if (fl.pre_bnd_pending && lb0 && !rs_bnd && red_defer_ok() &&
         path_choice(MMBA_PATH_PRE_SCHUR) == 1) {
         const RedSpec rs = epi_rows(pw, epi_ncol(*this), epi.do_xn, epi.do_gn);
-        launch_schur_obs(s, P, d_J, d_Lb, d_W, &rs, d_partial, d_scalar, d_gate);
+        launch_schur_obs(s, P, d_J, d_Lb, d_W, &rs, d_partial, d_scalar, d_gate, loads_first());
         fl.pre_sobs_pending = true;
     }
     fl.pre_jac_x = dx;
@@ -377,6 +383,7 @@
     const bool fuse = lm && ne_epilogue_fusable(P) && nrows == 0 && !b15;
     NeEpi epi;
     epi.probe = d_k2probe;
+    epi.loads_first = loads_first() ? 1 : 0;
     fl.lb0_valid = false;
     if (fuse) {
         epi = fused_epi(dx, *lm);
@@ -607,7 +614,7 @@
             launch_schur_obs_rs(s, PV, M, d_nloc, d_vobs, d_vcoff, d_J, d_Lb, d_W);
         else if (!ahead) {
             launch_schur_obs(s, P, d_J, d_Lb, d_W, fl.pend_red ? &pend_rs : nullptr, d_partial,
-                             d_scalar);
+                             d_scalar, nullptr, loads_first());
             fl.pend_red = false;
         }
     }
diff --git a/mayamatchmovesolver_amd/csrc/mmba_plan.cpp b/mayamatchmovesolver_amd/csrc/mmba_plan.cpp
--- a/mayamatchmovesolver_amd/csrc/mmba_plan.cpp
+++ b/mayamatchmovesolver_amd/csrc/mmba_plan.cpp
@@ -16,19 +16,20 @@
 
 Plan::~Plan() {
     if (d_k2probe) {
-        std::vector<long long> t(5 * (size_t)ncf);
+        constexpr int N = K2_PROBE_N;
+        std::vector<long long> t(N * (size_t)ncf);
         if (hipMemcpy(t.data(), d_k2probe, sizeof(long long) * t.size(), hipMemcpyDeviceToHost) ==
             hipSuccess) {
             long long t0 = LLONG_MAX, tend = 0;
             for (int c = 0; c < ncf; ++c)
-                if (t[5 * c]) {
-                    t0 = std::min(t0, t[5 * c]);
-                    tend = std::max(tend, t[5 * c + 3]);
+                if (t[N * c]) {
+                    t0 = std::min(t0, t[N * c]);
+                    tend = std::max(tend, t[N * c + 3]);
                 }
-            std::vector<double> st, stg, obs, tail, tot;
+            std::vector<double> st, stg, obs, tail, tot, sums, stor, epi;
             int per_xcc[16] = {};
             for (int c = 0; c < ncf; ++c) {
-                const long long *q = &t[5 * c];
+                const long long *q = &t[N * c];
                 if (!q[0]) continue;
                 st.push_back((q[0] - t0) / 100.);
                 stg.push_back((q[1] - q[0]) / 100.);
@@ -36,6 +37,11 @@
                 tail.push_back((q[3] - q[2]) / 100.);
                 tot.push_back((q[3] - q[0]) / 100.);
                 per_xcc[q[4] & 15]++;
+                if (q[6] && q[7]) {
+                    sums.push_back((q[6] - q[2]) / 100.);
+                    stor.push_back((q[7] - q[6]) / 100.);
+                    epi.push_back((q[3] - q[7]) / 100.);
+                }
             }
             auto pct = [](std::vector<double> v, double p) {
                 if (v.empty()) return 0.;
@@ -50,7 +56,10 @@
                          pct(obs, 1), pct(tail, 0), pct(tail, .5), pct(tail, 1), pct(tot, 0),
                          pct(tot, .5), pct(tot, 1));
             for (int x = 0; x < 8; ++x) std::fprintf(stderr, " %d", per_xcc[x]);
-            std::fprintf(stderr, "\n");
+            std::fprintf(stderr, "; tail: sums %.2f/%.2f/%.2f stores %.2f/%.2f/%.2f "
+                                 "epilogue %.2f/%.2f/%.2f\n",
+                         pct(sums, 0), pct(sums, .5), pct(sums, 1), pct(stor, 0), pct(stor, .5),
+                         pct(stor, 1), pct(epi, 0), pct(epi, .5), pct(epi, 1));
         }
     }
     if (d_probe && bs.use_bcr && bs.bcr.fflags && bs.bcr.nblk >= 2) {
@@ -1336,6 +1345,17 @@
         }
         d_bobs_rp = upload(rp);
     }
+    {
+        std::vector<int> sp(M);
+        bool fits = true;
+        for (int i = 0; i < M; ++i) {
+            const int cf = d_cf[i];
+            const int sv = cf_var_off[cf + 1] - cf_var_off[cf] - 1;
+            fits = fits && sv >= 0 && sv < 256;
+            sp[i] = sv | (cf_pc[cf] << 8) | (bnd_pb[d_bnd[i]] << 16);
+        }
+        D.obs_sp = fits ? upload(sp) : nullptr;
+    }
     D.cam_lpar_off = upload(cam_lpar_off);
     {
         bool any_inst = false;
@@ -1683,8 +1703,9 @@
         }
     if (band) setup_band();
     if (path_choice(MMBA_PATH_PROBE) == 2) {
-        d_k2probe = dalloc<long long>(5 * (size_t)std::max(ncf, 1));
-        MMBA_HIP(hipMemsetAsync(d_k2probe, 0, 5 * (size_t)std::max(ncf, 1) * sizeof(long long), s));
+        const size_t np = K2_PROBE_N * (size_t)std::max(ncf, 1);
+        d_k2probe = dalloc<long long>(np);
+        MMBA_HIP(hipMemsetAsync(d_k2probe, 0, np * sizeof(long long), s));
     }
     if (band && path_choice(MMBA_PATH_PROBE) == 1) {
         const size_t np = 8 + 4 * ((size_t)std::max(nR, 1) + 64);
diff --git a/mayamatchmovesolver_amd/csrc/mmba_plan.h b/mayamatchmovesolver_amd/csrc/mmba_plan.h
--- a/mayamatchmovesolver_amd/csrc/mmba_plan.h
+++ b/mayamatchmovesolver_amd/csrc/mmba_plan.h
@@ -365,6 +365,8 @@
                          const TrialRed &red = TrialRed());
     static constexpr bool kTrialRedFold = true;
     bool trial_red_fold() const;
+    static constexpr bool kLoadsFirst = true;
+    bool loads_first() const;
     void stage_slots();
     RedSpec pend_rs{};
     bool red_defer_ok() const;
diff --git a/mayamatchmovesolver_amd/csrc/mmba_wave_dev.h b/mayamatchmovesolver_amd/csrc/mmba_wave_dev.h
--- a/mayamatchmovesolver_amd/csrc/mmba_wave_dev.h
+++ b/mayamatchmovesolver_amd/csrc/mmba_wave_dev.h
@@ -49,6 +49,32 @@
     for (int off = 32; off > 0; off >>= 1) v += __shfl_xor(v, off);
     return v;
 }
+template <int CTRL>
+__device__ __forceinline__ double wave_dpp_mov(double v) {
+    int lo = __double2loint(v), hi = __double2hiint(v);
+    lo = __builtin_amdgcn_update_dpp(lo, lo, CTRL, 0xf, 0xf, false);
+    hi = __builtin_amdgcn_update_dpp(hi, hi, CTRL, 0xf, 0xf, false);
+    return __hiloint2double(hi, lo);
+}
+__device__ __forceinline__ double wave_sum_lane0(double v) {
+    {
+        const unsigned lo = (unsigned)__double2loint(v), hi = (unsigned)__double2hiint(v);
+        const auto a = __builtin_amdgcn_permlane32_swap(lo, lo, false, false);
+        const auto b = __builtin_amdgcn_permlane32_swap(hi, hi, false, false);
+        v += __hiloint2double((int)b[1], (int)a[1]);
+    }
+    {
+        const unsigned lo = (unsigned)__double2loint(v), hi = (unsigned)__double2hiint(v);
+        const auto a = __builtin_amdgcn_permlane16_swap(lo, lo, false, false);
+        const auto b = __builtin_amdgcn_permlane16_swap(hi, hi, false, false);
+        v += __hiloint2double((int)b[1], (int)a[1]);
+    }
+    v += wave_dpp_mov<0x128>(v);
+    v += wave_dpp_mov<0x104>(v);
+    v += wave_dpp_mov<0x4e>(v);
+    v += wave_dpp_mov<0xb1>(v);
+    return v;
+}
 __device__ __forceinline__ double wave_max(double v) {
 #pragma unroll
     for (int off = 32; off > 0; off >>= 1) v = fmax(v, __shfl_xor(v, off));
```
